# baek0203/multimodal_survival_prediction

Measured on AMD Instinct MI355X. Metric: patients/sec per epoch (training epoch of the K-fold job: fwd + Cox + gate entropy + bwd + clip + Adam; HBM-resident cohort, batches gathered on the device inside the timed region -- the same epoch fed from pinned host memory over PCIe: config.h2d), higher is better.
Workload: dtype f32

## Files before the change

include/mmsurv.h:

```cpp
#ifndef MMSURV_H
#define MMSURV_H
#include <stdint.h>
#include <stddef.h>

#ifndef HIP_INCLUDE_HIP_HIP_RUNTIME_API_H
typedef struct ihipStream_t* hipStream_t;
typedef struct ihipEvent_t* hipEvent_t;
#endif

#define MMS_OK 0
#define MMS_ERR_ARG (-1)
#define MMS_ERR_LAUNCH (-2)
#define MMS_MAX_GROUP 10

#ifdef __cplusplus
extern "C" {
#endif

typedef struct Dims3 { int D; int H; int W; } Dims3;

typedef struct MmsDnOpts {
    int out_features;
    int persist_b4;
    int persist_b3;
// ... 152 lines not shown
typedef struct MmsWgradMember {
    float* dw2;
    float* dw1;
    float* dgamma2; float* dbeta2;
    int model; int layer;
} MmsWgradMember;
typedef struct MmsWgradShape {
    int ld; int C0;
    int ms3; int ms1;
    int dw_layout;
    int count;
} MmsWgradShape;

typedef struct Conv1BwdP {
    const float* dyraw; int lddy;
    const float* y; int ldy;
    BnSrc bn_out; BnBwd bb_out; int has_bn_out;
    int M; int N;
    const float* x; int ldx; int K; BnSrc bn_in;
    const float* w;
    int pool; Dims3 in;
    float* dw;
    float* dbn; int lddbn;
    double* s1; double* s2;
    int msplit;
    float* dgamma_out; float* dbeta_out;
    int srep; int sstride;
    float* fuse_dx; int fuse_lddx; int fuse_accumulate;
    float* fuse_dgamma; float* fuse_dbeta;
    const unsigned* live;
} Conv1BwdP;

typedef struct BnBwdApplyP {
    const float* dbn; int lddbn;
    const float* x; int ldx;
    float* dx; int lddx;
    int M; int C; BnSrc bn; BnBwd bb; int accumulate;
    float* dgamma; float* dbeta;
    const unsigned* live;
} BnBwdApplyP;

typedef struct HeadBwdP {
    const float* dout; int lddout;
    const float* pooled;
    const float* slab; int ld; int C; int B; int V; BnSrc bn;
    const float* w; int N;
    float* dw; float* dbias;
    float* dgamma; float* dbeta;
    float* dslab; int ldd;
    double* ext_sums;
} HeadBwdP;

typedef struct PoolBwdP {
    const float* dslab; int ld;
    const uint8_t* argmax; Dims3 out; Dims3 in; int B;
    const float* y0; BnSrc bn;
    float* dbn;
    double* s1; double* s2;
    const int* coords;
    int srep; int sstride;
} PoolBwdP;

typedef struct Conv0BwdWP {
    const float* dbn; const float* y0; BnSrc bn; BnBwd bb;
    const float* x; Dims3 in; Dims3 out; const int* coords; int M;
    float* dw; int msplit;
    float* dgamma; float* dbeta;
    float* dw_rep; int nrep;
    const unsigned* live;
} Conv0BwdWP;

typedef struct Conv0BwdDataP {
    const float* dbn;
    BnSrc bn;
    const float* w;
    Dims3 in; Dims3 out;
    int M;
    float* dx;
} Conv0BwdDataP;

typedef struct FbConvP {
    const float* x; int Cin; Dims3 in; Dims3 out; int B;
    int has_bn; BnSrc bn;
    const float* w; const float* bias; int Cout;
    float* y;
    double* osum; double* osumsq;
    const float* dy;
    float* dw; float* dbias;
    float* dbn_in; double* s1; double* s2;
    int msplit;
} FbConvP;

typedef struct FbPoolP {
    const float* y; int C; int V; int B; BnSrc bn;
    float* out; int ldo;
    const float* dout; int lddout;
    float* dbn; double* s1; double* s2;
} FbPoolP;

typedef struct InProlog {
    int bn;
    const float* gamma; const float* beta;
    float* rmean; float* rvar; long long* nbt;
    float eps; float momentum;
    int train;
    float drop_p;
    const float* drop_mask;
    const uint32_t* rng;
    uint32_t stream_id;
} InProlog;

typedef struct LinearFwdP {
    const float* x; int ldx; int M; int K;
    InProlog pro;
    const float* w; const float* bias; int N;
    float* y; int ldy; int out_relu;
} LinearFwdP;

typedef struct LinearBwdP {
    const float* dy; int lddy;
    const float* y; int ldy;
    int out_relu;
    const float* x; int ldx; int M; int K; InProlog pro;
    const float* w; int N;
    float* dw; float* dbias;
    float* dx; int lddx;
    float* dgamma; float* dbeta;
} LinearBwdP;

typedef struct GateP {
    const float* feats; const float* mask; int M;
    const float* w1; const float* b1; const float* w2; const float* b2;
    float* hidden;
    float* gate;
    float* fused;
    const float* dfused;
    float ent_weight;
    const float* dgate_ext;
    float* dfeats;
    float* dw1; float* db1; float* dw2; float* db2;
    float* entropy;
} GateP;

typedef struct CoxP {
    const float* h; int ldh;
    const float* time; const float* event; const float* valid; int n;
    float scale;
    float* lse;
    float* dh; int lddh;
    float* out;
    int tie_mode;
    float* tie_frac;
} CoxP;

typedef struct CindexP {
    const float* h; const float* time; const float* event; int n;
    unsigned long long* counts;
} CindexP;

#define MMS_CBOOT_MAX_N 1048576
#define MMS_CBOOT_MAX_R 1048576
#define MMS_CBOOT_MAX_M 8
typedef struct CbootP {
    const int* hrank; int ldh; int M;
    const int* trank;
    const int* event;
    const int* stratum;
    int n;
    const signed char* w; int ldw; int R;
    long long* out;
    int pair_rule;
} CbootP;

#define MMS_GENE_SCREEN_MAX_G 4194240
typedef struct GeneScreenP {
    const float* x; int N; int ld;
    int G; int P;
    const int* off;
    const int* row;
    const double* coef;
    double* U; double* V;
} GeneScreenP;

#define MMS_COXNET_MAX_TOL 1.0
#define MMS_COXNET_MAX_ITER 100000000
typedef struct CoxnetP {
    const float* x; int N; int ld; int G;
    int nrow;
    const int* row; const int* event; const int* glast;
    int P;
    const int* mult;
    const double* lam; const double* alpha;
    const double* inv_scale;
    double* beta; double* trial; double* grad;
    double* f; double* step;
    int* iters; int* status;
    double* loss; double* nsum; double* kkt; double* obj;
    double* E; double* R;
    double* Gr;
    int* counter;
    double tol; int max_iter;
} CoxnetP;

#define MMS_LRSCAN_MAX_N 65535
#define MMS_LRSCAN_MAX_C 65535
#define MMS_LRSCAN_MAX_Q 16777215
typedef struct LogrankScanP {
    int n; int ldr; int Q;
    int maxc;
    const int* rank;
    const int* pflag;
    const double* coef;
    const int* coff;
    const int* cut;
    const int* cset;
    const int* at;
    double* chi2_max; int* arg_max; double* chi2_at;
    double* U; double* V;
    int* n_high; int* d_high;
    int ldo;
} LogrankScanP;

#define MMS_TD_MAX_H 64
#define MMS_TD_MAX_M 64
#define MMS_TD_MAX_N 4096
#define MMS_TD_MAX_R 16777215
typedef struct TdMetricsP {
    int n; int H; int M; int R;
    const int* trank; const int* event;
    const int* hcut;
    const int* rord; int ldr;
    const double* surv; int ldh;
    const signed char* w; int ldw;
    double* G; double* km;
    double* wcase; double* wctrl;
    double* brier; double* auc_num;
} TdMetricsP;

#define MMS_COXNEWTON_MAX_P 16
#define MMS_COXNEWTON_MAX_N 4096
#define MMS_COXNEWTON_MAX_S 64
#define MMS_COXNEWTON_MAX_Q 16777215
#define MMS_COXNEWTON_MAX_TOL 1e-3
#define MMS_COXNEWTON_MAX_ITER 1000
typedef struct CoxNewtonP {
    int n; int p; int R; int S;
    const double* x; int ldx;
    const int* event; const int* glast;
    const signed char* w; int ldw;
    const int* cmask;
    double tol; int max_iter; double beta_max;
    double* beta; double* se;
    double* loglik; double* loglik0;
    int* iters; int* status;
    double* info;
} CoxNewtonP;

typedef struct AdamP {
    float* p; float* g; float* m; float* v; long long n;
    const float* hyper;
    double* sumsq;
    float* step;
    const float* skip_flag;
    int adamw;
    float* acc; const float* cox_out; const float* entropy;
    int* rng;
    const long long* w2_off; float* const* w2_pack_b; float* const* w2_pack_f; int n_w2; uint64_t w2_fragmask;
} AdamP;

typedef struct LinBigP {
    const float* x; int ldx; int M; int K;
    const float* w; const float* bias; int N;
    float* y; int ldy; int out_relu;
    int has_bn; BnSrc bn;
    float* rmean; float* rvar; long long* nbt; float momentum;
    float drop_p; const float* drop_mask; const uint32_t* rng; uint32_t stream_id; int train;
    double* osum; double* osumsq;
    const float* dy; int lddy;
    float* dw; float* dbias; int msplit;
    int core_only;
    float* dbn; int lddbn;
    double* s1; double* s2;
    float* dx; int lddx;
    float* dgamma; float* dbeta;
} LinBigP;

typedef struct MixP {
    float* feats; int ld; int M;
    const float* mask; int ldm;
    int nseg;
    int seg_begin[4]; int seg_width[4];
    const float* bias[4];
    float* dfeats; int ldd;
    float* dbias[4];
} MixP;

typedef struct MoeP {
    int M; int F;
    int stage;
    const float* feats; int ldf;
    const float* mask; int ldm;
    const float* valid;
    float* valid_x;
    float* gin; int ldg;
    const float* h2; int ldh2;
    const float* w3; const float* b3;
// ... 46 lines not shown
} AffRec;
typedef struct AffP {
    const AffRec* rec;
    int stage_floats;
} AffP;

int mms_abi_sizeof(const char* name);
int mms_abi_version(void);

int mms_init_coords(int* coords, int B, int D, int H, int W, hipStream_t s);
int mms_conv0_fwd(const Conv0FwdP* p, hipStream_t s);
int mms_pool_fwd(const PoolFwdP* p, hipStream_t s);
int mms_conv1_fwd(const Conv1FwdP* p, hipStream_t s);
int mms_conv3_fwd(const Conv3FwdP* p, hipStream_t s);
int mms_head_fwd(const HeadFwdP* p, hipStream_t s);
int mms_conv3_bwd_data(const Conv3BwdDataP* p, hipStream_t s);
int mms_conv3_bwd_weight(const Conv3BwdWP* p, hipStream_t s);
int mms_conv1_bwd_data(const Conv1BwdP* p, hipStream_t s);
int mms_conv1_bwd_weight(const Conv1BwdP* p, hipStream_t s);
int mms_bn_bwd_apply(const BnBwdApplyP* p, hipStream_t s);
int mms_head_bwd(const HeadBwdP* p, hipStream_t s);
int mms_pool_bwd(const PoolBwdP* p, hipStream_t s);
int mms_conv0_bwd_weight(const Conv0BwdWP* p, hipStream_t s);
int mms_unpack_conv3_grads(const void* table_host, int nlayers, hipStream_t s);
int mms_pack_conv3(const float* w, float* wpf, float* wpb, hipStream_t s);
int mms_pack_conv3_frag(const float* w, float* wff, float* wfb, hipStream_t s);
int mms_pack_conv3_table(const void* table_dev, int nlayers, hipStream_t s);
int mms_bn_running_update(const void* table_dev, int n, float momentum, hipStream_t s);


int mms_fb_conv_fwd(const FbConvP* p, hipStream_t s);
int mms_fb_conv_bwd_w(const FbConvP* p, hipStream_t s);
int mms_fb_conv_bwd_x(const FbConvP* p, hipStream_t s);
int mms_fb_pool_fwd(const FbPoolP* p, hipStream_t s);
int mms_fb_pool_bwd(const FbPoolP* p, hipStream_t s);
int mms_fb_workspace_bytes(int B, int D, int H, int W, size_t* bytes);
int mms_fb_init(void* ws, int B, int D, int H, int W, const void* const* buffers, hipStream_t s);
int mms_fb_forward(void* ws, int B, int D, int H, int W, const float* x, const void* const* params,
                   const void* const* buffers, float* out, int ldo, int train, hipStream_t s);
int mms_fb_backward(void* ws, int B, int D, int H, int W, const float* x, const void* const* params,
                    const float* dout, int lddout, void* const* grads, hipStream_t s);
int mms_fb3_workspace_bytes(const int* widths, int B, int D, int H, int W, size_t* bytes);
int mms_fb3_init(void* ws, size_t ws_bytes, const int* widths, int B, int D, int H, int W, const void* const* buffers, hipStream_t s);
int mms_fb3_forward(void* ws, size_t ws_bytes, const int* widths, int B, int D, int H, int W, const float* x, const void* const* params,
                    const void* const* buffers, float* out, int ldo, int train, hipStream_t s);
int mms_fb3_backward(void* ws, size_t ws_bytes, const int* widths, int B, int D, int H, int W, const float* x, const void* const* params,
                     const float* dout, int lddout, void* const* grads, hipStream_t s);

int mms_conv0_bwd_data(const Conv0BwdDataP* p, hipStream_t s);
int mms_conv0_bwd_data_group(const Conv0BwdDataP* p, int ng, hipStream_t s);
int mms_dn121_input_grad(void* ws, int B, int D, int H, int W, const float* x, const void* const* params, const void* const* buffers,
                         const float* dout, int lddout, float* dx, const MmsDnOpts* opts, hipStream_t s);
int mms_fb3_input_grad(void* ws, size_t ws_bytes, const int* widths, int B, int D, int H, int W, const float* x, const void* const* params,
                       const void* const* buffers, const float* dout, int lddout, float* dx, hipStream_t s);
int mms_dn121_input_grad_group(int ng, void* const* ws, int B, int D, int H, int W, const float* const* x, const void* const* const* params,
                               const void* const* const* buffers, const float* const* dout, int lddout, float* const* dx,
                               const MmsDnOpts* opts, hipStream_t s);
int mms_fb3_input_grad_group(int ng, void* const* ws, size_t ws_bytes, const int* widths, int B, int D, int H, int W, const float* const* x,
                             const void* const* const* params, const void* const* const* buffers, const float* const* dout, int lddout,
                             float* const* dx, hipStream_t s);

typedef struct EnsP {
    const float* x[10];
    int K; size_t n;
    float* mean; float* spread;
} EnsP;
int mms_ensemble_reduce(const EnsP* p, hipStream_t s);

int mms_linear_fwd(const LinearFwdP* p, hipStream_t s);
int mms_linear_bwd(const LinearBwdP* p, hipStream_t s);
int mms_gate_fwd(const GateP* p, hipStream_t s);
int mms_gate_bwd(const GateP* p, hipStream_t s);
int mms_gate_entropy(const float* gate, int M, float scale, float* loss, float* dgate, hipStream_t s);
int mms_linear_big_fwd(const LinBigP* p, hipStream_t s);
int mms_linear_big_bwd_w(const LinBigP* p, hipStream_t s);
int mms_linear_big_bwd_x(const LinBigP* p, hipStream_t s);
int mms_bn1d_bwd_apply(const LinBigP* p, hipStream_t s);
int mms_missing_mix_fwd(const MixP* p, hipStream_t s);
int mms_missing_mix_bwd(const MixP* p, hipStream_t s);
int mms_cox_fwd_bwd(const CoxP* p, hipStream_t s);
int mms_moe_fwd(const MoeP* p, hipStream_t s);
int mms_moe_bwd(const MoeP* p, hipStream_t s);
int mms_cindex_counts(const CindexP* p, hipStream_t s);
int mms_cindex_boot(const CbootP* p, hipStream_t s);
int mms_gene_screen(const GeneScreenP* p, hipStream_t s);
int mms_logrank_scan(const LogrankScanP* p, hipStream_t s);
int mms_td_metrics(const TdMetricsP* p, hipStream_t s);
int mms_cox_newton(const CoxNewtonP* p, hipStream_t s);
int mms_coxnet_eval(const CoxnetP* p, hipStream_t s);
int mms_coxnet_iterate(const CoxnetP* p, int iters, hipStream_t s);
int mms_grad_sumsq(const AdamP* p, hipStream_t s);
int mms_clip_adam(const AdamP* p, hipStream_t s);
int mms_w2_pack(const AdamP* p, hipStream_t s);

int mms_ablation_build(void);
int mms_dn121_workspace_bytes(int B, int D, int H, int W, size_t* bytes);
int mms_dn121_region(int B, int D, int H, int W, const char* name, int index, size_t* off, size_t* bytes);
int mms_dn121_init(void* ws, int B, int D, int H, int W, const void* const* params, const void* const* buffers, const MmsDnOpts* opts, hipStream_t s);
int mms_dn121_w2_fragmask(int B, int D, int H, int W, const MmsDnOpts* opts, uint64_t* mask);
int mms_dn121_forward(void* ws, int B, int D, int H, int W, const float* x, const void* const* params,
                      const void* const* buffers, float* out, int ldo, int train, const MmsDnOpts* opts, hipStream_t s);
int mms_dn121_backward(void* ws, int B, int D, int H, int W, const float* x, const void* const* params,
                       const float* dout, int lddout, void* const* grads, const MmsDnOpts* opts, hipStream_t s);
typedef int (*mms_sync_fn)(void* user, double* base, int nrep, long rep_stride, int ncols, long pair_stride, hipStream_t s);
int mms_dn121_init_sync(void* ws, int B, int D, int H, int W, const void* const* params, const void* const* buffers, int bn_world,
                        const MmsDnOpts* opts, hipStream_t s);
int mms_dn121_forward_sync(void* ws, int B, int D, int H, int W, const float* x, const void* const* params,
                           const void* const* buffers, float* out, int ldo, int bn_world, mms_sync_fn hook, void* user,
                           const MmsDnOpts* opts, hipStream_t s);
int mms_dn121_backward_stage(void* ws, int B, int D, int H, int W, const float* x, const void* const* params,
                             const float* dout, int lddout, void* const* grads, int block_hi, int block_lo,
                             int bn_world, mms_sync_fn hook, void* user, const MmsDnOpts* opts, hipStream_t s);
int mms_head_bwd_sums(const HeadBwdP* p, hipStream_t s);
int mms_head_bwd_apply(const HeadBwdP* p, hipStream_t s);
int mms_dn121_backward_mt(void* ws, int B, int D, int H, int W, const float* x, const void* const* params,
                          const float* dout, int lddout, void* const* grads, const MmsDnOpts* opts, hipStream_t s, hipStream_t side,
                          hipEvent_t ev_fork, hipEvent_t ev_join);

int mms_ct_preprocess(const float* x, int inD, int inH, int inW, float* out, int oD, int oH, int oW, float* scratch, hipStream_t s);
int mms_rna_log_zscore(const float* counts, float* out, int n, int g, hipStream_t s);

int mms_conv0_fwd_group(const Conv0FwdP* p, int ng, const MmsDnOpts* opts, hipStream_t s);
int mms_conv0_fwd_group_zw(const Conv0FwdP* p, unsigned* const* zwords, int ng, const MmsDnOpts* opts, hipStream_t s);
int mms_pool_fwd_group(const PoolFwdP* p, int ng, hipStream_t s);
int mms_pool_act_group(const PoolActP* p, int ng, hipStream_t s);
int mms_conv1_fwd_group(const Conv1FwdP* p, int ng, const MmsDnOpts* opts, hipStream_t s);
int mms_conv3_fwd_group(const Conv3FwdP* p, int ng, const MmsDnOpts* opts, hipStream_t s);
int mms_head_fwd_group(const HeadFwdP* p, int ng, hipStream_t s);
int mms_conv3_bwd_data_group(const Conv3BwdDataP* p, int ng, const MmsDnOpts* opts, hipStream_t s);
int mms_conv3_bwd_weight_group(const Conv3BwdWP* p, int ng, const MmsDnOpts* opts, hipStream_t s);
int mms_conv3_bwd_weight_msplit(int M, int members, const MmsDnOpts* opts);
int mms_conv1_bwd_data_group(const Conv1BwdP* p, int ng, const MmsDnOpts* opts, hipStream_t s);
int mms_conv1_bwd_weight_group(const Conv1BwdP* p, int ng, hipStream_t s);
int mms_wgrad_tab_group(const MmsWgradModel* models, int nmodels, const MmsWgradMember* members, int nmembers,
                        const MmsWgradShape* shape, int which, hipStream_t s);
int mms_bn_bwd_apply_group(const BnBwdApplyP* p, int ng, hipStream_t s);
int mms_head_bwd_group(const HeadBwdP* p, int ng, hipStream_t s);
int mms_head_bwd_group_dup(const HeadBwdP* p, unsigned* const* live_out, const unsigned* const* zwords, int zbps, unsigned* const* dup_out,
                           int ng, hipStream_t s);
int mms_pool_bwd_group(const PoolBwdP* p, int ng, hipStream_t s);
int mms_conv0_bwd_weight_group(const Conv0BwdWP* p, int ng, const MmsDnOpts* opts, hipStream_t s);
int mms_pack_conv3_table_group(const void* const* tables_dev, int ng, int nlayers, hipStream_t s);
int mms_pack_conv3_table_group_ex(const void* const* tables_dev, int ng, int nlayers, uint64_t fragmask, hipStream_t s);
int mms_bn_running_update_group(const void* const* tables_dev, int ng, int n, float momentum, hipStream_t s);
int mms_missing_mix_fwd_group(const MixP* p, int ng, hipStream_t s);
int mms_missing_mix_bwd_group(const MixP* p, int ng, hipStream_t s);
int mms_gather_rows_group(const GatherP* p, int ng, hipStream_t s);
int mms_gather_aug_group(const GatherP* p, const AugP* a, int ng, hipStream_t s);
int mms_gather_affine_group(const GatherP* p, const AugP* a, const AffP* f, int ng, hipStream_t s);
int mms_unpack_conv3_grads_group(const float* const* scratch, float* const* const* dw, int ng, int nlayers, hipStream_t s);
int mms_zero_regions_group(void* const* regions_dev, int ng, size_t bytes, hipStream_t s);
int mms_linear_fwd_group(const LinearFwdP* p, int ng, hipStream_t s);
int mms_linear_bwd_group(const LinearBwdP* p, int ng, hipStream_t s);
int mms_gate_fwd_group(const GateP* p, int ng, hipStream_t s);
int mms_gate_bwd_group(const GateP* p, int ng, hipStream_t s);
int mms_cox_fwd_bwd_group(const CoxP* p, int ng, hipStream_t s);
int mms_moe_fwd_group(const MoeP* p, int ng, hipStream_t s);
int mms_moe_bwd_group(const MoeP* p, int ng, hipStream_t s);
int mms_grad_sumsq_group(const AdamP* p, int ng, hipStream_t s);
int mms_clip_adam_group(const AdamP* p, int ng, hipStream_t s);
int mms_w2_pack_group(const AdamP* p, int ng, hipStream_t s);
int mms_dn121_forward_group(int ng, void* const* ws, int B, int D, int H, int W, const float* const* x,
                            const void* const* const* params, const void* const* const* buffers, float* const* out,
                            int ldo, int train, const MmsDnOpts* opts, hipStream_t s);
int mms_dn121_backward_group(int ng, void* const* ws, int B, int D, int H, int W, const float* const* x,
                             const void* const* const* params, const float* const* dout, int lddout,
                             void* const* const* grads, const MmsDnOpts* opts, hipStream_t s);

int mms_fb_conv_fwd_group(const FbConvP* p, int ng, hipStream_t s);
int mms_fb_conv_bwd_w_group(const FbConvP* p, int ng, hipStream_t s);
int mms_fb_conv_bwd_x_group(const FbConvP* p, int ng, hipStream_t s);
int mms_fb_pool_fwd_group(const FbPoolP* p, int ng, hipStream_t s);
int mms_fb_pool_bwd_group(const FbPoolP* p, int ng, hipStream_t s);
int mms_fb_forward_group(int ng, void* const* ws, int B, int D, int H, int W, const float* const* x,
                         const void* const* const* params, const void* const* const* buffers, float* const* out,
                         int ldo, int train, hipStream_t s);
int mms_fb_backward_group(int ng, void* const* ws, int B, int D, int H, int W, const float* const* x,
                          const void* const* const* params, const float* const* dout, int lddout,
                          void* const* const* grads, hipStream_t s);
int mms_fb3_forward_group(int ng, void* const* ws, size_t ws_bytes, const int* widths, int B, int D, int H, int W, const float* const* x,
                          const void* const* const* params, const void* const* const* buffers, float* const* out,
                          int ldo, int train, hipStream_t s);
int mms_fb3_backward_group(int ng, void* const* ws, size_t ws_bytes, const int* widths, int B, int D, int H, int W, const float* const* x,
                           const void* const* const* params, const float* const* dout, int lddout,
                           void* const* const* grads, hipStream_t s);
int mms_img_tail_fwd_group(const FbPoolP* pool, const LinearFwdP* l1, const LinearFwdP* l2, int ng, hipStream_t s);
int mms_img_tail_bwd_group(const FbPoolP* pool, const LinearBwdP* l1, const LinearBwdP* l2, int ng, hipStream_t s);
int mms_img_forward_group(int ng, void* const* ws, size_t ws_bytes, const int* widths, int B, int D, int H, int W, const float* const* x,
                          const void* const* const* params, const void* const* const* buffers, float* const* out,
                          int ldo, int train, const LinearFwdP* l1, const LinearFwdP* l2, hipStream_t s);
int mms_img_backward_group(int ng, void* const* ws, size_t ws_bytes, const int* widths, int B, int D, int H, int W, const float* const* x,
                           const void* const* const* params, void* const* const* grads, const LinearBwdP* l1, const LinearBwdP* l2,
                           hipStream_t s);

#ifdef __cplusplus
}
#endif
#endif
```

multimodal_survival_prediction_amd/csrc/abi.hip:

```cpp
#include "common.h"
#include <string.h>

#define SZ(T) if (strcmp(name, #T) == 0) return (int)sizeof(T);
extern "C" int mms_abi_sizeof(const char* name) {
    SZ(Dims3) SZ(MmsDnOpts) SZ(BnSrc) SZ(BnBwd) SZ(Conv1FwdP) SZ(Conv3FwdP) SZ(Conv0FwdP) SZ(PoolFwdP) SZ(PoolActP) SZ(HeadFwdP)
    SZ(Conv3BwdDataP) SZ(Conv3BwdWP) SZ(Conv1BwdP) SZ(BnBwdApplyP) SZ(HeadBwdP) SZ(PoolBwdP) SZ(Conv0BwdWP) SZ(Conv0BwdDataP) SZ(InProlog) SZ(LinearFwdP) SZ(LinearBwdP) SZ(GateP) SZ(CoxP) SZ(CindexP) SZ(AdamP) SZ(FbConvP) SZ(FbPoolP) SZ(GatherP) SZ(AugRec) SZ(AugP) SZ(AffRec) SZ(AffP) SZ(MixP) SZ(LinBigP) SZ(MoeP) SZ(MmsWgradModel) SZ(MmsWgradMember) SZ(MmsWgradShape) SZ(EnsP) SZ(CbootP) SZ(GeneScreenP) SZ(CoxnetP) SZ(LogrankScanP) SZ(TdMetricsP) SZ(CoxNewtonP)
    return -1;
}
extern "C" int mms_abi_version(void) { return 3; }
extern "C" int mms_ablation_build(void) {
#if defined(MMS_ABLATE_STEP) || defined(MMS_ABLATE_SETUP) || defined(MMS_ABLATE_FLUSH) || defined(MMS_ABLATE_STATS) || defined(B4_TIMING) || defined(C3S_TIMING) || defined(C3M_TIMING)
    return 1;
#else
    return 0;
#endif
}
```

multimodal_survival_prediction_amd/csrc/heads.hip:

```cpp
#include "common.h"
#include "gather_rows.h"

template <int MM>
struct ColProlog {
    float xhat[MM], pre[MM], scale[MM];
    float mean, rstd, gamma;
    template <bool UPDATE_RUNNING>
    __device__ __forceinline__ void apply(const InProlog& pr, float (&x)[MM], int M, int k, int K) {
        if (pr.bn) {
            float mu, var;
            if (pr.train) {
                mu = 0;
#pragma unroll
                for (int m = 0; m < MM; ++m) if (m < M) mu += x[m];
                mu /= (float)M;
                var = 0;
#pragma unroll
                for (int m = 0; m < MM; ++m) if (m < M) { float d = x[m] - mu; var = fmaf(d, d, var); }
                var /= (float)M;
                if (UPDATE_RUNNING) {
                    const float unb = M > 1 ? var * (float)M / (float)(M - 1) : var;
                    pr.rmean[k] = (1.f - pr.momentum) * pr.rmean[k] + pr.momentum * mu;
                    pr.rvar[k] = (1.f - pr.momentum) * pr.rvar[k] + pr.momentum * unb;
                }
            } else {
                mu = pr.rmean[k]; var = pr.rvar[k];
            }
            mean = mu; rstd = 1.0f / sqrtf(var + pr.eps); gamma = pr.gamma[k];
            const float be = pr.beta[k];
#pragma unroll
            for (int m = 0; m < MM; ++m) {
                xhat[m] = (x[m] - mu) * rstd;
                pre[m] = fmaf(gamma, xhat[m], be);
                x[m] = fmaxf(pre[m], 0.f);
            }
        }
#pragma unroll
        for (int m = 0; m < MM; ++m) scale[m] = 1.f;
        if (pr.train && (pr.drop_mask || pr.drop_p > 0.f)) {
#pragma unroll
            for (int m = 0; m < MM; ++m) {
                if (m < M) {
                    scale[m] = pr.drop_mask ? pr.drop_mask[(size_t)m * K + k]
                                            : dropout_scale(pr.rng[0] + 0x9E3779B9u * pr.rng[1], pr.stream_id, (uint32_t)(m * K + k), pr.drop_p);
                    x[m] *= scale[m];
                }
            }
        }
    }
};

template <int MM, bool KS4>
__global__ __launch_bounds__(256) void linear_fwd_kernel(const Grp<LinearFwdP> grp) {
    const LinearFwdP& p = grp.p[blockIdx.z];
    __shared__ float red[4][MM];
    const int lane = threadIdx.x & 63, wave = threadIdx.x >> 6, n = KS4 ? (int)blockIdx.x : (int)blockIdx.x * 4 + wave;
    if (n >= p.N) return;
    constexpr int KSTEP = KS4 ? 256 : 64;
    const bool upd = (n == 0) && p.pro.bn && p.pro.train;
    float acc[MM];
#pragma unroll
    for (int m = 0; m < MM; ++m) acc[m] = 0.f;
    int kstart = lane + (KS4 ? 64 * wave : 0);
    const float* __restrict__ wr = p.w + (size_t)n * p.K;
    const float* __restrict__ xr = p.x;
    const bool plain = !p.pro.bn && !(p.pro.train && (p.pro.drop_mask || p.pro.drop_p > 0.f));
    constexpr int NU = MM <= 4 ? 8 : (MM <= 8 ? 4 : 2);
    for (; kstart + KSTEP * (NU - 1) < p.K; kstart += KSTEP * NU) {
        float w4[NU], x4[NU][MM];
#pragma unroll
        for (int u = 0; u < NU; ++u) {
            w4[u] = wr[kstart + KSTEP * u];
#pragma unroll
            for (int m = 0; m < MM; ++m) x4[u][m] = m < p.M ? xr[(size_t)m * p.ldx + kstart + KSTEP * u] : 0.f;
        }
#pragma unroll
        for (int u = 0; u < NU; ++u) {
            if (!plain) {
                ColProlog<MM> cp;
                if (upd) cp.template apply<true>(p.pro, x4[u], p.M, kstart + KSTEP * u, p.K); else cp.template apply<false>(p.pro, x4[u], p.M, kstart + KSTEP * u, p.K);
            }
#pragma unroll
            for (int m = 0; m < MM; ++m) acc[m] = fmaf(w4[u], x4[u][m], acc[m]);
        }
    }
    for (int k = kstart; k < p.K; k += KSTEP) {
        float x[MM];
#pragma unroll
        for (int m = 0; m < MM; ++m) x[m] = m < p.M ? xr[(size_t)m * p.ldx + k] : 0.f;
        ColProlog<MM> cp;
        if (upd) cp.template apply<true>(p.pro, x, p.M, k, p.K); else cp.template apply<false>(p.pro, x, p.M, k, p.K);
        const float w = wr[k];
#pragma unroll
        for (int m = 0; m < MM; ++m) acc[m] = fmaf(w, x[m], acc[m]);
    }
    if (upd && lane == 0 && (!KS4 || wave == 0) && p.pro.nbt) *p.pro.nbt += 1;
    const float b = p.bias ? p.bias[n] : 0.f;
#pragma unroll
    for (int m = 0; m < MM; ++m) acc[m] = wave_sum(acc[m]);
    if constexpr (KS4) {
        if (lane == 0) {
#pragma unroll
            for (int m = 0; m < MM; ++m) red[wave][m] = acc[m];
        }
        __syncthreads();
        if (wave != 0) return;
#pragma unroll
        for (int m = 0; m < MM; ++m) acc[m] = red[0][m] + red[1][m] + red[2][m] + red[3][m];
    }
    if (lane == 0) {
#pragma unroll
        for (int m = 0; m < MM; ++m)
            if (m < p.M) {
                const float v = acc[m] + b;
                p.y[(size_t)m * p.ldy + n] = p.out_relu ? fmaxf(v, 0.f) : v;
            }
    }
}

template <int MM>
static int launch_linear_fwd(const Grp<LinearFwdP>& a, int ng, hipStream_t s) {
    if (a.p[0].K >= 2048) MMS_LAUNCH((linear_fwd_kernel<MM, true>), dim3(a.p[0].N, 1, ng), dim3(256), 0, s, a);
    else MMS_LAUNCH((linear_fwd_kernel<MM, false>), dim3((a.p[0].N + 3) / 4, 1, ng), dim3(256), 0, s, a);
    return mms_check_launch();
}
extern "C" int mms_linear_fwd_group(const LinearFwdP* pp, int ng, hipStream_t s) {
    Grp<LinearFwdP> a;
    if (!grp_fill(a, pp, ng, 1)) return MMS_ERR_ARG;
    const LinearFwdP& p = *pp;
    if (p.M <= 0 || p.M > 32 || p.N <= 0 || p.K <= 0) return MMS_ERR_ARG;
    if (p.pro.bn && p.pro.train && p.M < 2) return MMS_ERR_ARG;
    for (int g = 1; g < ng; ++g) {
        const LinearFwdP& q = pp[g];
        if (q.M != p.M || q.N != p.N || q.K != p.K || q.pro.bn != p.pro.bn || q.pro.train != p.pro.train) return MMS_ERR_ARG;
    }
    if (p.M <= 4) return launch_linear_fwd<4>(a, ng, s);
    if (p.M <= 8) return launch_linear_fwd<8>(a, ng, s);
    if (p.M <= 16) return launch_linear_fwd<16>(a, ng, s);
    return launch_linear_fwd<32>(a, ng, s);
}
MMS_SINGLE(mms_linear_fwd, LinearFwdP)

template <int MM, bool KS4>
__global__ __launch_bounds__(256) void linear_bwd_w_kernel(const Grp<LinearBwdP> grp) {
    const LinearBwdP& p = grp.p[blockIdx.z];
    const int lane = threadIdx.x & 63, wave = threadIdx.x >> 6, n = KS4 ? (int)blockIdx.x : (int)blockIdx.x * 4 + wave;
    if (n >= p.N) return;
    constexpr int KSTEP = KS4 ? 256 : 64;
    float dz[MM], db = 0.f;
#pragma unroll
    for (int m = 0; m < MM; ++m) {
        float g = 0.f;
        if (m < p.M) {
            g = p.dy[(size_t)m * p.lddy + n];
            if (p.out_relu && !(p.y[(size_t)m * p.ldy + n] > 0.f)) g = 0.f;
        }
        dz[m] = g; db += g;
    }
    if (lane == 0 && (!KS4 || wave == 0) && p.dbias) p.dbias[n] += db;
    constexpr int NU = MM <= 4 ? 8 : 2;
    float* __restrict__ dwr = p.dw + (size_t)n * p.K;
    const float* __restrict__ xr = p.x;
    int k0 = lane + (KS4 ? 64 * wave : 0);
    for (; k0 + KSTEP * (NU - 1) < p.K; k0 += KSTEP * NU) {
        float d0[NU], xx[NU][MM];
#pragma unroll
        for (int u = 0; u < NU; ++u) {
            d0[u] = dwr[k0 + KSTEP * u];
#pragma unroll
            for (int m = 0; m < MM; ++m) xx[u][m] = m < p.M ? xr[(size_t)m * p.ldx + k0 + KSTEP * u] : 0.f;
        }
#pragma unroll
        for (int u = 0; u < NU; ++u) {
            ColProlog<MM> cp;
            cp.template apply<false>(p.pro, xx[u], p.M, k0 + KSTEP * u, p.K);
            float a = 0.f;
#pragma unroll
            for (int m = 0; m < MM; ++m) a = fmaf(dz[m], xx[u][m], a);
            dwr[k0 + KSTEP * u] = d0[u] + a;
        }
    }
    for (int k = k0; k < p.K; k += KSTEP) {
        float x[MM];
#pragma unroll
        for (int m = 0; m < MM; ++m) x[m] = m < p.M ? p.x[(size_t)m * p.ldx + k] : 0.f;
        ColProlog<MM> cp;
        cp.template apply<false>(p.pro, x, p.M, k, p.K);
        float a = 0.f;
#pragma unroll
        for (int m = 0; m < MM; ++m) a = fmaf(dz[m], x[m], a);
        p.dw[(size_t)n * p.K + k] += a;
    }
}

template <int MM>
__global__ __launch_bounds__(256) void linear_bwd_x_kernel(const Grp<LinearBwdP> grp) {
    const LinearBwdP& p = grp.p[blockIdx.z];
    __shared__ float dzs[MM][128];
    __shared__ float red[3][MM][64];
    const int lane = threadIdx.x & 63, wave = threadIdx.x >> 6;
    const int k = blockIdx.x * 64 + lane;
    const int N = p.N, K = p.K;
    const float* __restrict__ wk = p.w + (k < K ? k : K - 1);
    float acc[MM];
#pragma unroll
    for (int m = 0; m < MM; ++m) acc[m] = 0.f;
    for (int nb = 0; nb < N; nb += 128) {
        __syncthreads();
        for (int idx = threadIdx.x; idx < MM * 128; idx += 256) {
            const int m = idx >> 7, n = nb + (idx & 127);
            float g = 0.f;
            if (m < p.M && n < N) {
                g = p.dy[(size_t)m * p.lddy + n];
                if (p.out_relu && !(p.y[(size_t)m * p.ldy + n] > 0.f)) g = 0.f;
            }
            dzs[m][idx & 127] = g;
        }
        __syncthreads();
        if (nb + 32 * wave < N) {
#pragma unroll
            for (int h = 0; h < 2; ++h) {
                float wv[16];
#pragma unroll
                for (int j = 0; j < 16; ++j) {
                    const int n = nb + 32 * wave + 16 * h + j;
                    wv[j] = wk[(size_t)(n < N ? n : N - 1) * K];
                }
#pragma unroll
                for (int j = 0; j < 16; ++j)
#pragma unroll
                    for (int m = 0; m < MM; ++m) acc[m] = fmaf(dzs[m][32 * wave + 16 * h + j], wv[j], acc[m]);
            }
        }
    }
    if (wave > 0) {
#pragma unroll
        for (int m = 0; m < MM; ++m) red[wave - 1][m][lane] = acc[m];
    }
    __syncthreads();
    if (wave > 0 || k >= K) return;
#pragma unroll
    for (int m = 0; m < MM; ++m) acc[m] += red[0][m][lane] + red[1][m][lane] + red[2][m][lane];
    float x[MM];
#pragma unroll
    for (int m = 0; m < MM; ++m) x[m] = m < p.M ? p.x[(size_t)m * p.ldx + k] : 0.f;
    ColProlog<MM> cp;
    cp.template apply<false>(p.pro, x, p.M, k, p.K);
    float dxv[MM];
    if (p.pro.bn) {
        float s1 = 0.f, s2 = 0.f, dpre[MM];
#pragma unroll
        for (int m = 0; m < MM; ++m) {
            dpre[m] = (m < p.M && cp.pre[m] > 0.f) ? acc[m] * cp.scale[m] : 0.f;
            s1 += dpre[m]; s2 = fmaf(dpre[m], cp.xhat[m], s2);
        }
        if (p.dgamma) { p.dgamma[k] += s2; p.dbeta[k] += s1; }
        const float gr = cp.gamma * cp.rstd, m1 = s1 / (float)p.M, m2 = s2 / (float)p.M;
#pragma unroll
        for (int m = 0; m < MM; ++m)
            dxv[m] = p.pro.train ? gr * (dpre[m] - m1 - cp.xhat[m] * m2) : gr * dpre[m];
    } else {
#pragma unroll
        for (int m = 0; m < MM; ++m) dxv[m] = acc[m] * cp.scale[m];
    }
#pragma unroll
    for (int m = 0; m < MM; ++m) if (m < p.M) p.dx[(size_t)m * p.lddx + k] = dxv[m];
}

template <int MM>
static int launch_linear_bwd(const Grp<LinearBwdP>& a, int ng, hipStream_t s) {
    const LinearBwdP& p = a.p[0];
    if (p.dw) {
        if (p.K >= 2048) MMS_LAUNCH((linear_bwd_w_kernel<MM, true>), dim3(p.N, 1, ng), dim3(256), 0, s, a);
        else MMS_LAUNCH((linear_bwd_w_kernel<MM, false>), dim3((p.N + 3) / 4, 1, ng), dim3(256), 0, s, a);
    }
    if (p.dx) MMS_LAUNCH(linear_bwd_x_kernel<MM>, dim3((p.K + 63) / 64, 1, ng), dim3(256), 0, s, a);
    return mms_check_launch();
}
extern "C" int mms_linear_bwd_group(const LinearBwdP* pp, int ng, hipStream_t s) {
    Grp<LinearBwdP> a;
    if (!grp_fill(a, pp, ng, 1)) return MMS_ERR_ARG;
    const LinearBwdP& p = *pp;
    if (p.M <= 0 || p.M > 32 || p.N <= 0 || p.K <= 0) return MMS_ERR_ARG;
    for (int g = 1; g < ng; ++g) {
        const LinearBwdP& q = pp[g];
        if (q.M != p.M || q.N != p.N || q.K != p.K || (q.dw == nullptr) != (p.dw == nullptr) || (q.dx == nullptr) != (p.dx == nullptr)) return MMS_ERR_ARG;
    }
    if (p.M <= 4) return launch_linear_bwd<4>(a, ng, s);
    if (p.M <= 8) return launch_linear_bwd<8>(a, ng, s);
    if (p.M <= 16) return launch_linear_bwd<16>(a, ng, s);
    return launch_linear_bwd<32>(a, ng, s);
}
MMS_SINGLE(mms_linear_bwd, LinearBwdP)

#define GATE_F 288
#define GATE_IN 291
__device__ __forceinline__ int gate_seg(int t) { return t < 128 ? 0 : (t < 256 ? 1 : 2); }

__global__ __launch_bounds__(256) void gate_fwd_kernel(const Grp<GateP> grp) {
    const GateP& p = grp.p[blockIdx.z];
    __shared__ float G[GATE_IN + 1], h[64], g[3];
    const int m = blockIdx.x, t = threadIdx.x, lane = t & 63, wave = t >> 6;
    for (int i = t; i < GATE_IN; i += 256)
        G[i] = i < GATE_F ? p.feats[(size_t)m * GATE_F + i] * p.mask[m * 3 + gate_seg(i)] : p.mask[m * 3 + (i - GATE_F)];
    __syncthreads();
    for (int j = wave * 16; j < wave * 16 + 16; ++j) {
        float a = 0.f;
        for (int k = lane; k < GATE_IN; k += 64) a = fmaf(p.w1[j * GATE_IN + k], G[k], a);
        a = wave_sum(a);
        if (lane == 0) { h[j] = fmaxf(a + p.b1[j], 0.f); p.hidden[m * 64 + j] = h[j]; }
    }
    __syncthreads();
    if (wave == 0) {
        float l[3];
#pragma unroll
        for (int c = 0; c < 3; ++c) l[c] = wave_sum(p.w2[c * 64 + lane] * h[lane]) + p.b2[c];
        if (lane == 0) {
            const float mx = fmaxf(l[0], fmaxf(l[1], l[2]));
            const float e0 = expf(l[0] - mx), e1 = expf(l[1] - mx), e2 = expf(l[2] - mx), inv = 1.f / (e0 + e1 + e2);
            g[0] = e0 * inv; g[1] = e1 * inv; g[2] = e2 * inv;
            float ent = 0.f;
#pragma unroll
            for (int c = 0; c < 3; ++c) { p.gate[m * 3 + c] = g[c]; ent += g[c] * logf(g[c] + 1e-8f); }
            if (p.entropy) atomicAdd(p.entropy, ent / (float)p.M);
        }
    }
    __syncthreads();
    for (int i = t; i < GATE_F; i += 256) p.fused[(size_t)m * GATE_F + i] = G[i] * g[gate_seg(i)];
}

__global__ __launch_bounds__(256) void gate_bwd_kernel(const Grp<GateP> grp) {
    const GateP& p = grp.p[blockIdx.z];
    __shared__ float G[GATE_IN + 1], h[64], g[3], dgs[3], dl[3], dhp[64], red[4][3];
    const int m = blockIdx.x, t = threadIdx.x, lane = t & 63, wave = t >> 6;
    for (int i = t; i < GATE_IN; i += 256)
        G[i] = i < GATE_F ? p.feats[(size_t)m * GATE_F + i] * p.mask[m * 3 + gate_seg(i)] : p.mask[m * 3 + (i - GATE_F)];
    if (t < 64) h[t] = p.hidden[m * 64 + t];
    if (t < 3) g[t] = p.gate[m * 3 + t];
    __syncthreads();
    float part[3] = {0.f, 0.f, 0.f};
    for (int i = t; i < GATE_F; i += 256) part[gate_seg(i)] += p.dfused[(size_t)m * GATE_F + i] * G[i];
#pragma unroll
    for (int c = 0; c < 3; ++c) { float v = wave_sum(part[c]); if (lane == 0) red[wave][c] = v; }
    __syncthreads();
    if (t == 0) {
        float dg[3], dot = 0.f;
#pragma unroll
        for (int c = 0; c < 3; ++c) {
            dg[c] = red[0][c] + red[1][c] + red[2][c] + red[3][c];
            if (p.ent_weight != 0.f) dg[c] += p.ent_weight / (float)p.M * (logf(g[c] + 1e-8f) + g[c] / (g[c] + 1e-8f));
            if (p.dgate_ext) dg[c] += p.dgate_ext[m * 3 + c];
            dot += g[c] * dg[c];
        }
#pragma unroll
        for (int c = 0; c < 3; ++c) { dl[c] = g[c] * (dg[c] - dot); atomicAdd(&p.db2[c], dl[c]); }
    }
    __syncthreads();
    if (t < 64) {
        float dh = 0.f;
#pragma unroll
        for (int c = 0; c < 3; ++c) { dh = fmaf(dl[c], p.w2[c * 64 + t], dh); atomicAdd(&p.dw2[c * 64 + t], dl[c] * h[t]); }
        dhp[t] = h[t] > 0.f ? dh : 0.f;
        atomicAdd(&p.db1[t], dhp[t]);
    }
    __syncthreads();
    for (int idx = t; idx < 64 * GATE_IN; idx += 256) {
        const int j = idx / GATE_IN, k = idx % GATE_IN;
        atomicAdd(&p.dw1[idx], dhp[j] * G[k]);
    }
    for (int i = t; i < GATE_F; i += 256) {
        float dG = 0.f;
        for (int j = 0; j < 64; ++j) dG = fmaf(dhp[j], p.w1[j * GATE_IN + i], dG);
        const int sg = gate_seg(i);
        p.dfeats[(size_t)m * GATE_F + i] = (p.dfused[(size_t)m * GATE_F + i] * g[sg] + dG) * p.mask[m * 3 + sg];
    }
}
#define GATE_TR 8
template <bool SPLIT>
__global__ __launch_bounds__(256) void gate_bwd_tiled_kernel(const Grp<GateP> grp) {
    const GateP& p = grp.p[blockIdx.z];
    __shared__ float G[GATE_IN + 1], h[64], g[3], dl[3], dhp[64], red[4][3];
    const int t = threadIdx.x, lane = t & 63, wave = t >> 6;
    const int role = SPLIT ? (int)blockIdx.y : 0;
    const bool do_acc = !SPLIT || role == 0, do_feats = !SPLIT || role > 0;
    int m_lo = blockIdx.x * GATE_TR, m_hi = m_lo + GATE_TR < p.M ? m_lo + GATE_TR : p.M;
    if (SPLIT && role > 0) { m_lo += role - 1; if (m_lo >= m_hi) return; m_hi = m_lo + 1; }
    const bool two = t < GATE_IN - 256;
    float a0[64], a1[64];
#pragma unroll
    for (int j = 0; j < 64; ++j) { a0[j] = 0.f; a1[j] = 0.f; }
    float ab1 = 0.f, aw2[3] = {0.f, 0.f, 0.f}, ab2[3] = {0.f, 0.f, 0.f};
    for (int m = m_lo; m < m_hi; ++m) {
        __syncthreads();
        for (int i = t; i < GATE_IN; i += 256)
            G[i] = i < GATE_F ? p.feats[(size_t)m * GATE_F + i] * p.mask[m * 3 + gate_seg(i)] : p.mask[m * 3 + (i - GATE_F)];
        if (t < 64) h[t] = p.hidden[m * 64 + t];
        if (t < 3) g[t] = p.gate[m * 3 + t];
        __syncthreads();
        float part[3] = {0.f, 0.f, 0.f};
        for (int i = t; i < GATE_F; i += 256) part[gate_seg(i)] += p.dfused[(size_t)m * GATE_F + i] * G[i];
#pragma unroll
        for (int c = 0; c < 3; ++c) { float v = wave_sum(part[c]); if (lane == 0) red[wave][c] = v; }
        __syncthreads();
        if (t == 0) {
            float dg[3], dot = 0.f;
#pragma unroll
            for (int c = 0; c < 3; ++c) {
                dg[c] = red[0][c] + red[1][c] + red[2][c] + red[3][c];
                if (p.ent_weight != 0.f) dg[c] += p.ent_weight / (float)p.M * (logf(g[c] + 1e-8f) + g[c] / (g[c] + 1e-8f));
                if (p.dgate_ext) dg[c] += p.dgate_ext[m * 3 + c];
                dot += g[c] * dg[c];
            }
#pragma unroll
            for (int c = 0; c < 3; ++c) { dl[c] = g[c] * (dg[c] - dot); ab2[c] += dl[c]; }
        }
        __syncthreads();
        if (t < 64) {
            float dh = 0.f;
#pragma unroll
            for (int c = 0; c < 3; ++c) { dh = fmaf(dl[c], p.w2[c * 64 + t], dh); aw2[c] = fmaf(dl[c], h[t], aw2[c]); }
            dhp[t] = h[t] > 0.f ? dh : 0.f;
            ab1 += dhp[t];
        }
        __syncthreads();
        if (do_acc) {
            const float g0 = G[t], g1 = two ? G[256 + t] : 0.f;
#pragma unroll
            for (int j = 0; j < 64; ++j) { const float d = dhp[j]; a0[j] = fmaf(d, g0, a0[j]); a1[j] = fmaf(d, g1, a1[j]); }
        }
        if (do_feats)
            for (int i = t; i < GATE_F; i += 256) {
                float dG = 0.f;
                for (int j = 0; j < 64; ++j) dG = fmaf(dhp[j], p.w1[j * GATE_IN + i], dG);
                const int sg = gate_seg(i);
                p.dfeats[(size_t)m * GATE_F + i] = (p.dfused[(size_t)m * GATE_F + i] * g[sg] + dG) * p.mask[m * 3 + sg];
            }
    }
    if (!do_acc) return;
#pragma unroll
    for (int j = 0; j < 64; ++j) {
        atomicAdd(&p.dw1[j * GATE_IN + t], a0[j]);
        if (two) atomicAdd(&p.dw1[j * GATE_IN + 256 + t], a1[j]);
    }
    if (t < 64) {
        atomicAdd(&p.db1[t], ab1);
#pragma unroll
        for (int c = 0; c < 3; ++c) atomicAdd(&p.dw2[c * 64 + t], aw2[c]);
    }
    if (t == 0) {
#pragma unroll
        for (int c = 0; c < 3; ++c) atomicAdd(&p.db2[c], ab2[c]);
    }
}
__global__ void gate_entropy_kernel(const float* gate, int M, float scale, float* loss, float* dgate) {
    const int m = blockIdx.x * 64 + threadIdx.x;
    float e = 0.f;
    if (m < M) {
#pragma unroll
        for (int c = 0; c < 3; ++c) {
            const float g = gate[m * 3 + c];
            e += g * logf(g + 1e-8f);
            if (dgate) dgate[m * 3 + c] = scale / (float)M * (logf(g + 1e-8f) + g / (g + 1e-8f));
        }
    }
    e = wave_sum(e);
    if (threadIdx.x == 0 && loss) atomicAdd(loss, e / (float)M);
}
extern "C" int mms_gate_entropy(const float* gate, int M, float scale, float* loss, float* dgate, hipStream_t s) {
    if (M <= 0) return MMS_ERR_ARG;
    MMS_LAUNCH(gate_entropy_kernel, dim3((M + 63) / 64), dim3(64), 0, s, gate, M, scale, loss, dgate);
    return mms_check_launch();
}

static bool gate_group(Grp<GateP>& a, const GateP* pp, int ng) {
    if (!grp_fill(a, pp, ng, 1) || pp->M <= 0) return false;
    for (int g = 1; g < ng; ++g) if (pp[g].M != pp->M) return false;
    return true;
}
extern "C" int mms_gate_fwd_group(const GateP* pp, int ng, hipStream_t s) {
    Grp<GateP> a;
    if (!gate_group(a, pp, ng)) return MMS_ERR_ARG;
    MMS_LAUNCH(gate_fwd_kernel, dim3(pp->M, 1, ng), dim3(256), 0, s, a);
    return mms_check_launch();
}
extern "C" int mms_gate_bwd_group(const GateP* pp, int ng, hipStream_t s) {
    Grp<GateP> a;
    if (!gate_group(a, pp, ng)) return MMS_ERR_ARG;
    if (pp->M <= GATE_TR) MMS_LAUNCH(gate_bwd_tiled_kernel<true>, dim3(1, 1 + pp->M, ng), dim3(256), 0, s, a);
    else if (pp->M > 32) MMS_LAUNCH(gate_bwd_tiled_kernel<false>, dim3((pp->M + GATE_TR - 1) / GATE_TR, 1, ng), dim3(256), 0, s, a);
    else MMS_LAUNCH(gate_bwd_kernel, dim3(pp->M, 1, ng), dim3(256), 0, s, a);
    return mms_check_launch();
}
MMS_SINGLE(mms_gate_fwd, GateP)
MMS_SINGLE(mms_gate_bwd, GateP)

__device__ __forceinline__ bool cox_valid(const CoxP& p, int i) { return p.valid == nullptr || p.valid[i] != 0.f; }

__global__ __launch_bounds__(256) void cox_lse_kernel(const Grp<CoxP> grp) {
    const CoxP& p = grp.p[blockIdx.z];
    const int lane = threadIdx.x & 63, i = blockIdx.x * 4 + (threadIdx.x >> 6);
    if (i >= p.n) return;
    if (!cox_valid(p, i)) { if (lane == 0) { p.lse[i] = 0.f; if (p.tie_mode == 1) p.tie_frac[i] = -1.f; } return; }
    const float ti = p.time[i];
    float mx = -INFINITY;
    for (int j = lane; j < p.n; j += 64)
        if (cox_valid(p, j) && p.time[j] >= ti) mx = fmaxf(mx, p.h[(size_t)j * p.ldh]);
    mx = wave_max(mx);
    float s = 0.f;
    if (p.tie_mode != 1) {
        for (int j = lane; j < p.n; j += 64)
            if (cox_valid(p, j) && p.time[j] >= ti) s += expf(p.h[(size_t)j * p.ldh] - mx);
        s = wave_sum(s);
        if (lane == 0) p.lse[i] = mx + logf(s);
        return;
    }
    float st = 0.f, m = 0.f, l = 0.f;
    for (int j = lane; j < p.n; j += 64)
        if (cox_valid(p, j)) {
            const float tj = p.time[j];
            if (tj >= ti) {
                const float e = expf(p.h[(size_t)j * p.ldh] - mx);
                s += e;
                if (tj == ti && p.event[j] != 0.f) { st += e; m += 1.f; l += j < i ? 1.f : 0.f; }
            }
        }
    s = wave_sum(s); st = wave_sum(st); m = wave_sum(m); l = wave_sum(l);
    if (lane == 0) {
        const bool ev = p.event[i] != 0.f;
        const float f = ev ? l / m : 0.f;
        p.lse[i] = mx + logf(s - f * st);
        p.tie_frac[i] = ev ? f : -1.f;
    }
}

__global__ __launch_bounds__(256) void cox_grad_kernel(const Grp<CoxP> grp) {
    const CoxP& p = grp.p[blockIdx.z];
    __shared__ float red[8];
    const int lane = threadIdx.x & 63, wave = threadIdx.x >> 6, k = blockIdx.x * 4 + wave;
    const bool efron = p.tie_mode == 1;
    float nv = 0.f, ne = 0.f, ls = 0.f, nd = 0.f;
    for (int j = threadIdx.x; j < p.n; j += 256)
        if (cox_valid(p, j)) {
            nv += 1.f;
            if (p.event[j] != 0.f) {
                ne += 1.f; ls += p.h[(size_t)j * p.ldh] - p.lse[j];
                if (efron && p.tie_frac[j] == 0.f) nd += 1.f;
            }
        }
    nv = wave_sum(nv); ne = wave_sum(ne); ls = wave_sum(ls); nd = wave_sum(nd);
    if (lane == 0) { red[wave] = nv; red[4 + wave] = ne; }
    __syncthreads();
    nv = red[0] + red[1] + red[2] + red[3]; ne = red[4] + red[5] + red[6] + red[7];
    __syncthreads();
    if (lane == 0) { red[wave] = ls; red[4 + wave] = nd; }
    __syncthreads();
    ls = red[0] + red[1] + red[2] + red[3]; nd = red[4] + red[5] + red[6] + red[7];
    const bool usable = nv >= 2.f && ne > 0.f;
    const float denom = efron ? nd : ne + 1e-8f;
    if (blockIdx.x == 0 && threadIdx.x == 0) {
        p.out[0] = usable ? -ls / denom : 0.f;
        p.out[1] = usable ? 1.f : 0.f;
    }
    if (k >= p.n || p.dh == nullptr) return;
    float gsum = 0.f;
    if (usable && cox_valid(p, k)) {
        const float tk = p.time[k], hk = p.h[(size_t)k * p.ldh];
        const bool ek = p.event[k] != 0.f;
        for (int i = lane; i < p.n; i += 64)
            if (cox_valid(p, i) && p.event[i] != 0.f && p.time[i] <= tk) {
                float w = 1.f;
                if (efron && ek && p.time[i] == tk) w -= p.tie_frac[i];
                gsum += w * expf(hk - p.lse[i]);
            }
        gsum = wave_sum(gsum);
        if (lane == 0) p.dh[(size_t)k * p.lddh] = -p.scale * ((ek ? 1.f : 0.f) - gsum) / denom;
    } else if (lane == 0) {
        p.dh[(size_t)k * p.lddh] = 0.f;
    }
}
extern "C" int mms_cox_fwd_bwd_group(const CoxP* pp, int ng, hipStream_t s) {
    Grp<CoxP> a;
    if (!grp_fill(a, pp, ng, 1)) return MMS_ERR_ARG;
    const CoxP& p = *pp;
    for (int g = 0; g < ng; ++g)
        if (pp[g].n != p.n || pp[g].n <= 0 || !pp[g].lse || !pp[g].out || pp[g].tie_mode < 0 || pp[g].tie_mode > 1 || (pp[g].tie_mode == 1 && !pp[g].tie_frac)) return MMS_ERR_ARG;
    MMS_LAUNCH(cox_lse_kernel, dim3((p.n + 3) / 4, 1, ng), dim3(256), 0, s, a);
    MMS_LAUNCH(cox_grad_kernel, dim3((p.n + 3) / 4, 1, ng), dim3(256), 0, s, a);
    return mms_check_launch();
}
MMS_SINGLE(mms_cox_fwd_bwd, CoxP)

__global__ __launch_bounds__(256) void cindex_kernel(const CindexP p) {
    const int lane = threadIdx.x & 63, i = blockIdx.x * 4 + (threadIdx.x >> 6);
    if (i >= p.n || p.event[i] != 1.f) return;
    const float ti = p.time[i], hi = p.h[i];
    unsigned conc = 0, tied = 0, perm = 0;
    for (int j = lane; j < p.n; j += 64)
        if (p.time[j] > ti) {
            ++perm;
            const float hj = p.h[j];
            conc += hi > hj; tied += hi == hj;
        }
#pragma unroll
    for (int o = 32; o > 0; o >>= 1) { conc += __shfl_xor(conc, o, 64); tied += __shfl_xor(tied, o, 64); perm += __shfl_xor(perm, o, 64); }
    if (lane == 0) {
        atomicAdd(&p.counts[0], (unsigned long long)conc);
        atomicAdd(&p.counts[1], (unsigned long long)tied);
        atomicAdd(&p.counts[2], (unsigned long long)perm);
    }
}
extern "C" int mms_cindex_counts(const CindexP* pp, hipStream_t s) {
    if (pp->n <= 0) return MMS_ERR_ARG;
    MMS_LAUNCH(cindex_kernel, dim3((pp->n + 3) / 4), dim3(256), 0, s, *pp);
    return mms_check_launch();
}

__global__ __launch_bounds__(256) void grad_sumsq_kernel(const Grp<AdamP> grp) {
    const AdamP& p = grp.p[blockIdx.z];
    __shared__ double red[4];
    const long long n4 = p.n >> 2, stride = (long long)gridDim.x * 256;
    float a = 0.f, a1 = 0.f, a2 = 0.f, a3 = 0.f;
    long long i = (long long)blockIdx.x * 256 + threadIdx.x;
    for (; i + 3 * stride < n4; i += 4 * stride) {
        const float4 g0 = ((const float4*)p.g)[i], g1 = ((const float4*)p.g)[i + stride], g2 = ((const float4*)p.g)[i + 2 * stride],
                     g3 = ((const float4*)p.g)[i + 3 * stride];
        a = fmaf(g0.x, g0.x, a); a = fmaf(g0.y, g0.y, a); a = fmaf(g0.z, g0.z, a); a = fmaf(g0.w, g0.w, a);
        a1 = fmaf(g1.x, g1.x, a1); a1 = fmaf(g1.y, g1.y, a1); a1 = fmaf(g1.z, g1.z, a1); a1 = fmaf(g1.w, g1.w, a1);
        a2 = fmaf(g2.x, g2.x, a2); a2 = fmaf(g2.y, g2.y, a2); a2 = fmaf(g2.z, g2.z, a2); a2 = fmaf(g2.w, g2.w, a2);
        a3 = fmaf(g3.x, g3.x, a3); a3 = fmaf(g3.y, g3.y, a3); a3 = fmaf(g3.z, g3.z, a3); a3 = fmaf(g3.w, g3.w, a3);
    }
    for (; i < n4; i += stride) {
        const float4 g = ((const float4*)p.g)[i];
        a = fmaf(g.x, g.x, a); a = fmaf(g.y, g.y, a); a = fmaf(g.z, g.z, a); a = fmaf(g.w, g.w, a);
    }
    a += a1 + a2 + a3;
    if (blockIdx.x == 0 && threadIdx.x < (p.n & 3)) { const float g = p.g[(n4 << 2) + threadIdx.x]; a = fmaf(g, g, a); }
    const double t = block_sum_d((double)a, red);
    if (threadIdx.x == 0) {
        atomicAdd(p.sumsq, t);
        if (blockIdx.x == 0) {
            if (p.skip_flag == nullptr || *p.skip_flag != 0.f) p.step[0] += 1.f;
            if (p.acc) {
                if (p.cox_out) { p.acc[0] += p.cox_out[0] * p.cox_out[1]; p.acc[1] += p.cox_out[1]; }
                if (p.entropy) p.acc[2] += p.entropy[0];
                p.acc[3] += 1.f;
            }
            if (p.rng) p.rng[1] += 1;
        }
    }
}
constexpr int W2N = 32 * 27 * 128;
__global__ __launch_bounds__(256) void clip_adam_kernel(const Grp<AdamP> grp) {
    const AdamP& p = grp.p[blockIdx.z];
    __shared__ float c[6];
    if (p.skip_flag != nullptr && *p.skip_flag == 0.f) return;
    if (threadIdx.x == 0) {
        const double lr = p.hyper[0], b1 = p.hyper[1], b2 = p.hyper[2], wd = p.hyper[4], maxn = p.hyper[5];
        const double t = p.step[0];
        const double norm = sqrt(*p.sumsq);
        double coef = maxn / (norm + 1e-6);
        if (coef > 1.0) coef = 1.0;
        if (maxn <= 0.0) coef = 1.0;
        const double bc1 = 1.0 - pow(b1, t), bc2 = 1.0 - pow(b2, t);
        c[0] = (float)coef; c[1] = (float)(lr / bc1); c[2] = (float)(1.0 / sqrt(bc2));
        c[3] = (float)(1.0 - lr * wd); c[4] = (float)wd;
    }
    __syncthreads();
    const float coef = c[0], step_size = c[1], inv_sqrt_bc2 = c[2], decay = c[3], wd = c[4];
    const float b1 = p.hyper[1], b2 = p.hyper[2], eps = p.hyper[3];
    const long long stride = (long long)gridDim.x * 256;
    __shared__ long long vp[64];
    const int nw = p.n_w2;
    if ((int)threadIdx.x < nw) vp[threadIdx.x] = p.w2_off[threadIdx.x] - (long long)threadIdx.x * W2N;
    if (nw) __syncthreads();
    const long long nv = p.n - (long long)nw * W2N;
    for (long long j = (long long)blockIdx.x * 256 + threadIdx.x; j < nv; j += stride) {
        int lo = 0, hi = nw;
        while (lo < hi) { const int mid = (lo + hi) >> 1; if (vp[mid] <= j) lo = mid + 1; else hi = mid; }
        const long long i = j + (long long)lo * W2N;
        float w = p.p[i], g = p.g[i] * coef;
        if (p.adamw) w *= decay; else g = fmaf(wd, w, g);
        const float m = fmaf(b1, p.m[i], (1.f - b1) * g);
        const float v = fmaf(b2, p.v[i], (1.f - b2) * g * g);
        p.m[i] = m; p.v[i] = v;
        p.p[i] = w - step_size * m / (sqrtf(v) * inv_sqrt_bc2 + eps);
    }
}

constexpr int W2P = 132;

template <bool UPDATE>
__global__ __launch_bounds__(256) void w2_adam_pack_kernel(const Grp<AdamP> grp) {
    const AdamP& p = grp.p[blockIdx.z];
    const int tap = blockIdx.x, layer = blockIdx.y, tid = threadIdx.x;
    __shared__ __attribute__((aligned(16))) float t[32 * W2P];
    __shared__ float c[6];
    if (UPDATE) {
        if (p.skip_flag != nullptr && *p.skip_flag == 0.f) return;
        if (tid == 0) {
            const double lr = p.hyper[0], b1 = p.hyper[1], b2 = p.hyper[2], wd = p.hyper[4], maxn = p.hyper[5];
            const double st = p.step[0];
            const double norm = sqrt(*p.sumsq);
            double coef = maxn / (norm + 1e-6);
            if (coef > 1.0) coef = 1.0;
            if (maxn <= 0.0) coef = 1.0;
            const double bc1 = 1.0 - pow(b1, st), bc2 = 1.0 - pow(b2, st);
            c[0] = (float)coef; c[1] = (float)(lr / bc1); c[2] = (float)(1.0 / sqrt(bc2));
            c[3] = (float)(1.0 - lr * wd); c[4] = (float)wd;
        }
        __syncthreads();
    }
    const size_t base = (size_t)p.w2_off[layer];
    float4 w4[4];
    size_t off[4];
#pragma unroll
    for (int j = 0; j < 4; ++j) {
        const int idx4 = tid + 256 * j, co = idx4 >> 5, c4 = idx4 & 31;
        off[j] = base + ((size_t)co * 27 + tap) * 128 + 4 * c4;
        w4[j] = *(const float4*)(p.p + off[j]);
    }
    if (UPDATE) {
        float4 g4[4], m4[4], v4[4];
#pragma unroll
        for (int j = 0; j < 4; ++j) { g4[j] = *(const float4*)(p.g + off[j]); m4[j] = *(const float4*)(p.m + off[j]); v4[j] = *(const float4*)(p.v + off[j]); }
        const float coef = c[0], step_size = c[1], inv_sqrt_bc2 = c[2], decay = c[3], wd = c[4];
        const float b1 = p.hyper[1], b2 = p.hyper[2], eps = p.hyper[3];
        auto upd = [&](float& w, float g, float& m, float& v) {
            g *= coef;
            if (p.adamw) w *= decay; else g = fmaf(wd, w, g);
            m = fmaf(b1, m, (1.f - b1) * g);
            v = fmaf(b2, v, (1.f - b2) * g * g);
            w = w - step_size * m / (sqrtf(v) * inv_sqrt_bc2 + eps);
        };
#pragma unroll
        for (int j = 0; j < 4; ++j) {
            upd(w4[j].x, g4[j].x, m4[j].x, v4[j].x); upd(w4[j].y, g4[j].y, m4[j].y, v4[j].y);
            upd(w4[j].z, g4[j].z, m4[j].z, v4[j].z); upd(w4[j].w, g4[j].w, m4[j].w, v4[j].w);
            *(float4*)(p.p + off[j]) = w4[j]; *(float4*)(p.m + off[j]) = m4[j]; *(float4*)(p.v + off[j]) = v4[j];
        }
    }
#pragma unroll
    for (int j = 0; j < 4; ++j) {
        const int idx4 = tid + 256 * j, co = idx4 >> 5, c4 = idx4 & 31;
        *(float4*)(t + co * W2P + 4 * c4) = w4[j];
    }
    __syncthreads();
    const bool frag = (p.w2_fragmask >> layer) & 1ull;
    float4* pb = (float4*)p.w2_pack_b[layer];
    if (frag) {
        float4* dst = pb + (size_t)tap * 1024;
#pragma unroll
        for (int j = 0; j < 4; ++j) {
            const int idx4 = tid + 256 * j, q = idx4 >> 6, lane = idx4 & 63;
            const int cin = ((q >> 1) << 4) | (lane & 15), co0 = ((q & 1) << 4) | ((lane >> 4) << 2);
            dst[idx4] = make_float4(t[co0 * W2P + cin], t[(co0 + 1) * W2P + cin], t[(co0 + 2) * W2P + cin], t[(co0 + 3) * W2P + cin]);
        }
        float4* df = (float4*)p.w2_pack_f[layer] + (size_t)tap * 1024;
#pragma unroll
        for (int j = 0; j < 4; ++j) {
            const int idx4 = tid + 256 * j, q = idx4 >> 6, lane = idx4 & 63;
            const int c4 = ((q >> 1) << 2) | (lane >> 4), co = ((q & 1) << 4) | (lane & 15);
            df[idx4] = *(const float4*)(t + co * W2P + 4 * c4);
        }
    } else {
#pragma unroll
        for (int j = 0; j < 4; ++j) {
            const int idx4 = tid + 256 * j, cin = idx4 >> 3, co0 = (idx4 & 7) << 2;
            pb[((size_t)cin * 27 + tap) * 8 + (idx4 & 7)] =
                make_float4(t[co0 * W2P + cin], t[(co0 + 1) * W2P + cin], t[(co0 + 2) * W2P + cin], t[(co0 + 3) * W2P + cin]);
        }
    }
}



static bool adam_group(Grp<AdamP>& a, const AdamP* pp, int ng) {
    if (!grp_fill(a, pp, ng, 1) || pp->n <= 0) return false;
    for (int g = 0; g < ng; ++g) {
        const AdamP& p = pp[g];
        if (p.n != pp->n || p.n_w2 != pp->n_w2 || p.w2_fragmask != pp->w2_fragmask || p.n_w2 < 0 || p.n_w2 > 64) return false;
        if (p.n_w2 && (!p.w2_off || !p.w2_pack_b || (p.w2_fragmask && !p.w2_pack_f) || (((uintptr_t)p.p | (uintptr_t)p.g | (uintptr_t)p.m | (uintptr_t)p.v) & 15))) return false;
    }
    return true;
}
extern "C" int mms_grad_sumsq_group(const AdamP* pp, int ng, hipStream_t s) {
    Grp<AdamP> a;
    if (!adam_group(a, pp, ng)) return MMS_ERR_ARG;
    long long blocks = (pp->n / 16 + 255) / 256;
    if (blocks > 1024) blocks = 1024;
    if (blocks < 1) blocks = 1;
    MMS_LAUNCH(grad_sumsq_kernel, dim3((unsigned)blocks, 1, ng), dim3(256), 0, s, a);
    return mms_check_launch();
}
extern "C" int mms_clip_adam_group(const AdamP* pp, int ng, hipStream_t s) {
    Grp<AdamP> a;
    if (!adam_group(a, pp, ng)) return MMS_ERR_ARG;
    long long blocks = (pp->n + 255) / 256;
    if (blocks > 4096) blocks = 4096;
    MMS_LAUNCH(clip_adam_kernel, dim3((unsigned)blocks, 1, ng), dim3(256), 0, s, a);
    if (pp->n_w2 > 0) MMS_LAUNCH(w2_adam_pack_kernel<true>, dim3(27, pp->n_w2, ng), dim3(256), 0, s, a);
    return mms_check_launch();
}
extern "C" int mms_w2_pack_group(const AdamP* pp, int ng, hipStream_t s) {
    Grp<AdamP> a;
    if (!adam_group(a, pp, ng)) return MMS_ERR_ARG;
    if (pp->n_w2 > 0) MMS_LAUNCH(w2_adam_pack_kernel<false>, dim3(27, pp->n_w2, ng), dim3(256), 0, s, a);
    return mms_check_launch();
}
MMS_SINGLE(mms_grad_sumsq, AdamP)
MMS_SINGLE(mms_clip_adam, AdamP)
MMS_SINGLE(mms_w2_pack, AdamP)

__global__ __launch_bounds__(256) void gather_rows_kernel(const Grp<GatherP> grp) {
    const GatherP& p = grp.p[blockIdx.z];
    const int b = blockIdx.y;
    if (b >= p.B) return;
    const long long row = p.idx[b];
    const int t0 = blockIdx.x * 256 + threadIdx.x, stride = gridDim.x * 256;
    for (int s = 0; s < p.nsrc; ++s) {
        const float* src = p.src[s] + (size_t)row * p.src_ld[s];
        float* dst = p.dst[s] + (size_t)b * p.dst_ld[s];
        const int w = p.width[s];
        const bool absent = p.present[s] && p.present[s][(size_t)row * p.present_ld[s]] == 0.f;
        if ((w & 3) == 0 && (((uintptr_t)src | (uintptr_t)dst) & 15) == 0) {
            if (absent) { for (int i = t0; i < (w >> 2); i += stride) ((float4*)dst)[i] = make_float4(0.f, 0.f, 0.f, 0.f); }
            else {
                int i = t0;
                for (; i + 3 * stride < (w >> 2); i += 4 * stride) {
                    const float4 a = ((const float4*)src)[i], b = ((const float4*)src)[i + stride], c = ((const float4*)src)[i + 2 * stride],
                                 d = ((const float4*)src)[i + 3 * stride];
                    ((float4*)dst)[i] = a; ((float4*)dst)[i + stride] = b; ((float4*)dst)[i + 2 * stride] = c; ((float4*)dst)[i + 3 * stride] = d;
                }
                for (; i < (w >> 2); i += stride) ((float4*)dst)[i] = ((const float4*)src)[i];
            }
        } else {
            for (int i = t0; i < w; i += stride) dst[i] = absent ? 0.f : src[i];
        }
    }
}
extern "C" int mms_gather_rows_group(const GatherP* pp, int ng, hipStream_t s) {
    Grp<GatherP> a;
    if (!grp_fill(a, pp, ng, 1)) return MMS_ERR_ARG;
    int wmax = 0;
    for (int g = 0; g < ng; ++g) {
        const GatherP& q = pp[g];
        if (q.B != pp->B || q.B <= 0 || !q.idx || q.nsrc < 1 || q.nsrc > 8) return MMS_ERR_ARG;
        for (int i = 0; i < q.nsrc; ++i) {
            if (!q.src[i] || !q.dst[i] || q.width[i] <= 0) return MMS_ERR_ARG;
            if (q.width[i] > wmax) wmax = q.width[i];
        }
    }
    int blocks = (wmax / 4 + 1023) / 1024;
    if (blocks < 1) blocks = 1;
    if (blocks > 64) blocks = 64;
    MMS_LAUNCH(gather_rows_kernel, dim3(blocks, pp->B, ng), dim3(256), 0, s, a);
    return mms_check_launch();
}

#define AUG_TILE4 1024

__global__ __launch_bounds__(256) void gather_aug_kernel(const Grp<GatherP> grp, const AugGrp ag) {
    __shared__ float4 tile[AUG_TILE4];
    const GatherP& p = grp.p[blockIdx.z];
    const AugK& k = ag.k[blockIdx.z];
    const int b = blockIdx.y;
    if (b >= p.B) return;
    const long long row = p.idx[b];
    const AugRec r = k.rec[b];
    const int t0 = blockIdx.x * 256 + threadIdx.x, stride = gridDim.x * 256;
    const bool ident_i = r.scale == 1.f && r.offset == 0.f;
    const bool ident = ident_i && (r.flip & 7) == 0 && r.dz == 0 && r.dy == 0 && r.dx == 0;
    for (int s = 0; s < p.nsrc; ++s) {
        const float* src;
        float* dst;
        if (gather_plain_source(p, k.meta, r.drop, s, row, b, ident, t0, stride, src, dst)) continue;
        const int w = p.width[s];
        const int D = ag.D, H = ag.H, W = ag.W;
        const int dz = max(-D, min(D, r.dz)), dy = max(-H, min(H, r.dy)), dx = max(-W, min(W, r.dx));
        const bool fD = r.flip & 1, fH = r.flip & 2, fW = r.flip & 4;
        if ((W & 3) == 0 && W <= 4 * AUG_TILE4 && (((uintptr_t)src | (uintptr_t)dst) & 15) == 0) {
            const int W4 = W >> 2, LT = AUG_TILE4 / W4, nlines = D * H, ntiles = (nlines + LT - 1) / LT;
            for (int t = blockIdx.x; t < ntiles; t += gridDim.x) {
                const int l0 = t * LT, n4 = min(LT, nlines - l0) * W4;
                float4 v[4];
#pragma unroll
                for (int u = 0; u < 4; ++u) {
                    const int j = threadIdx.x + u * 256;
                    v[u] = make_float4(0.f, 0.f, 0.f, 0.f);
                    if (j < n4) {
                        const int l = l0 + j / W4, xq = j - (j / W4) * W4;
                        const int z = l / H, y = l - z * H;
                        const int sz = (fD ? D - 1 - z : z) - dz, sy = (fH ? H - 1 - y : y) - dy;
                        if (sz >= 0 && sz < D && sy >= 0 && sy < H)
                            v[u] = ((const float4*)src)[(size_t)(sz * H + sy) * W4 + xq];
                    }
                }
#pragma unroll
                for (int u = 0; u < 4; ++u) { const int j = threadIdx.x + u * 256; if (j < n4) tile[j] = v[u]; }
                __syncthreads();
                const float* tf = (const float*)tile;
#pragma unroll
                for (int u = 0; u < 4; ++u) {
                    const int j = threadIdx.x + u * 256;
                    if (j < n4) {
                        const int ll = j / W4, x0 = (j - ll * W4) * 4;
                        float o[4];
#pragma unroll
                        for (int e = 0; e < 4; ++e) {
                            const int x = x0 + e, sx = (fW ? W - 1 - x : x) - dx;
                            const float q = (sx >= 0 && sx < W) ? tf[ll * W + sx] : 0.f;
                            o[e] = ident_i ? q : fmaf(r.scale, q, r.offset);
                        }
                        ((float4*)dst)[(size_t)l0 * W4 + j] = make_float4(o[0], o[1], o[2], o[3]);
                    }
                }
                __syncthreads();
            }
        } else {
            for (int i = t0; i < w; i += stride) {
                const int x = i % W, l = i / W, y = l % H, z = l / H;
                const int sz = (fD ? D - 1 - z : z) - dz, sy = (fH ? H - 1 - y : y) - dy, sx = (fW ? W - 1 - x : x) - dx;
                const float q = (sz >= 0 && sz < D && sy >= 0 && sy < H && sx >= 0 && sx < W) ? src[((size_t)sz * H + sy) * W + sx] : 0.f;
                dst[i] = ident_i ? q : fmaf(r.scale, q, r.offset);
            }
        }
    }
}
extern "C" int mms_gather_aug_group(const GatherP* pp, const AugP* aa, int ng, hipStream_t s) {
    Grp<GatherP> a;
    if (!grp_fill(a, pp, ng, 1) || !aa) return MMS_ERR_ARG;
    AugGrp ag = {};
    int blocks = 0;
    if (!gather_aug_args(pp, aa, ng, ag, blocks)) return MMS_ERR_ARG;
    MMS_LAUNCH(gather_aug_kernel, dim3(blocks, pp->B, ng), dim3(256), 0, s, a, ag);
    return mms_check_launch();
}

__global__ __launch_bounds__(256) void missing_mix_kernel(const Grp<MixP> grp, int bwd) {
    const MixP& p = grp.p[blockIdx.z];
    const int j = blockIdx.x * 256 + threadIdx.x;
    int s = -1;
    for (int t = 0; t < p.nseg; ++t) if (j >= p.seg_begin[t] && j < p.seg_begin[t] + p.seg_width[t]) s = t;
    if (s < 0) return;
    const int jl = j - p.seg_begin[s];
    if (!bwd) {
        const float b = p.bias[s][jl];
// ... 37 lines not shown
```

multimodal_survival_prediction_amd/engine.py:

```python
import ctypes
import os

import torch
import torch.nn as nn

from . import _lib, ops

_S = _lib.structs



def check_train_batch(B, bn_world=1):
    if B * max(int(bn_world), 1) <= 1:
        raise ValueError("Expected more than 1 value per channel when training: a batch of 1 patient cannot be normalised by the "
                         "heads' BatchNorm1d layers (torch raises the same in the reference's train_epoch; choose a batch size / "
                         "fold split without a tail of 1)")

class _Lin:

    def __init__(self, lin, src, dst, out_relu, pro_bn=None, pro_drop=None, need_dx=True):
        self.lin, self.src, self.dst, self.out_relu = lin, src, dst, out_relu
        self.pro_bn, self.pro_drop, self.need_dx = pro_bn, pro_drop, need_dx


# ... 387 lines not shown
            P.gate = ops.gate_params(P.buf["feats"], P.mask, g1.weight, g1.bias, g2.weight, g2.bias, P.hidden, P.gatew,
                                     P.buf["fused"], P.dbuf["fused"], self.ent_weight, P.dbuf["feats"],
                                     gmap[id(g1.weight)], gmap[id(g1.bias)], gmap[id(g2.weight)], gmap[id(g2.bias)],
                                     self.entropy)
        P.mix = None
        if prog.get("mix") is not None:
            mx = prog["mix"]
            P.mask2 = torch.ones(B, len(mx["segs"]), device=dev)
            M = _S()["MixP"]()
            fe, dfe = P.buf["feats"], P.dbuf["feats"]
            M.feats, M.ld, M.M = fe.data_ptr(), fe.stride(0), B
            M.mask, M.ldm, M.nseg = P.mask2.data_ptr(), P.mask2.stride(0), len(mx["segs"])
            M.dfeats, M.ldd = dfe.data_ptr(), dfe.stride(0)
            for i, ((b0, w), bias) in enumerate(zip(mx["segs"], mx["biases"])):
                M.seg_begin[i], M.seg_width[i] = b0, w
                M.bias[i], M.dbias[i] = bias.data_ptr(), gmap[id(bias)].data_ptr()
            P.mix = M
        P.moe = None
        if prog.get("moe") is not None:
            self._plan_moe(P, gmap)
        hz = P.buf["hz"]
        ens_valid = P.valid_x[0] if P.moe is not None else P.valid
        P.cox = _S()["CoxP"](hz.data_ptr(), hz.stride(0), P.time.data_ptr(), P.event.data_ptr(), ens_valid.data_ptr(), B, 1.0,
                             P.lse.data_ptr(), P.dbuf["hz"].data_ptr(), P.dbuf["hz"].stride(0), P.cox_out.data_ptr(), self.tie_mode,
                             P.tie_frac.data_ptr())
        P.cox_eval_out = torch.zeros(2, device=self.device)
        P.cox_eval = _S()["CoxP"](hz.data_ptr(), hz.stride(0), P.time.data_ptr(), P.event.data_ptr(), ens_valid.data_ptr(), B, 1.0,
                                  P.lse.data_ptr(), None, 1, P.cox_eval_out.data_ptr(), self.tie_mode, P.tie_frac.data_ptr())
        book = dict(acc=self.acc, cox_out=P.cox_out, entropy=self.entropy, rng=self.rng)
        w2 = self.w2 if (self.w2 is not None and self.w2["fragmask"] is not None) else None
        if self.w2 is not None and w2 is None:
            raise RuntimeError("create the engine's first plan with the encoder (packed conv2 storage needs the volume size)")
        P.adam = ops.adam_params(self.flat, self.gflat, self.m, self.v, self.hyper, self.sumsq, self.step_count,
                                 None, self.adamw, w2=w2, **book)
        P.adam_skip = ops.adam_params(self.flat, self.gflat, self.m, self.v, self.hyper, self.sumsq, self.step_count,
                                      P.cox_out[1:], self.adamw, w2=w2, **book)
        P.graphs = {}
        self.plans[key] = P
        return P

    def _plan_moe(self, P, gmap):
        mo, B, dev, S = self.prog["moe"], P.B, self.device, _S()
        F = mo["F"]
        P.gatew = torch.zeros(B, 3, device=dev)
        P.fused = torch.zeros(B, F, device=dev)
        P.valid_x = torch.ones(4, B, device=dev)
        P.cox_outs = torch.zeros(4, 2, device=dev)
        P.lse4, P.frac4 = torch.zeros(4, B, device=dev), torch.zeros(4, B, device=dev)
        fe, dfe, hz, dhz = P.buf["feats"], P.dbuf["feats"], P.buf["hz"], P.dbuf["hz"]
        gin, dgin, h2, dh2 = P.buf["gin"], P.dbuf["gin"], P.buf["g2"], P.dbuf["g2"]
        out, ens = mo["out"], mo["ensemble"]

        def block(stage):
            q = S["MoeP"]()
            q.M, q.F, q.stage = B, F, stage
            q.feats, q.ldf, q.mask, q.ldm = fe.data_ptr(), fe.stride(0), P.mask.data_ptr(), P.mask.stride(0)
            q.valid, q.valid_x = P.valid.data_ptr(), P.valid_x.data_ptr()
            q.gin, q.ldg, q.h2, q.ldh2 = gin.data_ptr(), gin.stride(0), h2.data_ptr(), h2.stride(0)
            q.w3, q.b3 = out.weight.data_ptr(), out.bias.data_ptr()
            for e, L in enumerate(mo["experts"]):
                q.wx[e], q.bx[e] = L.weight.data_ptr(), L.bias.data_ptr()
                q.dwx[e], q.dbx[e] = gmap[id(L.weight)].data_ptr(), gmap[id(L.bias)].data_ptr()
            q.we, q.be = ens.weight.data_ptr(), ens.bias.data_ptr()
            q.hz, q.ldhz, q.gate, q.fused = hz.data_ptr(), hz.stride(0), P.gatew.data_ptr(), P.fused.data_ptr()
            q.dhz, q.lddhz, q.dh2, q.lddh2 = dhz.data_ptr(), dhz.stride(0), dh2.data_ptr(), dh2.stride(0)
            q.dgin, q.lddg, q.dfeats, q.lddf = dgin.data_ptr(), dgin.stride(0), dfe.data_ptr(), dfe.stride(0)
            q.dw3, q.db3 = gmap[id(out.weight)].data_ptr(), gmap[id(out.bias)].data_ptr()
            q.dwe, q.dbe = gmap[id(ens.weight)].data_ptr(), gmap[id(ens.bias)].data_ptr()
            q.cox_outs, q.expert_weight, q.loss_out = P.cox_outs.data_ptr(), self.expert_weight, P.cox_out.data_ptr()
            return q
        P.moe = [block(0), block(1)]
        P.moe_bwd = [block(0), block(1)]
        lam = self.expert_weight
        cox = (S["CoxP"] * 4)()
        for c in range(4):
            valid = P.valid_x[c]
            cox[c] = S["CoxP"](hz[:, c].data_ptr(), hz.stride(0), P.time.data_ptr(), P.event.data_ptr(), valid.data_ptr(), B,
                               1.0 if c == 0 else lam, P.lse4[c].data_ptr(), dhz[:, c].data_ptr(), dhz.stride(0), P.cox_outs[c].data_ptr(),
                               self.tie_mode, P.frac4[c].data_ptr())
        P.cox4 = cox

    def _cox_step(self, P):
        if P.moe is not None:
            _lib.check(self.lib.mms_cox_fwd_bwd_group(P.cox4, 4, ops.stream()), "mms_cox_fwd_bwd_group")
        else:
            _lib.check(self.lib.mms_cox_fwd_bwd(ctypes.byref(P.cox), ops.stream()), "mms_cox_fwd_bwd")

    def _plan_big(self, P, gmap):
        prog, B, dev = self.prog, P.B, self.device
        S, ptr = _S()["LinBigP"], ops.ptr
        widths = {L.src: L.lin.in_features for L in prog["lins"] if L.pro_bn is not None}
        off, o = {}, 0
        for name, k in widths.items():
            off[name] = o
            o += 4 * k
        P.big_stats = torch.zeros(max(o, 1), dtype=torch.float64, device=dev)
        P.big_dbn = torch.zeros(B, max(list(widths.values()) + [4]), device=dev)
        st = lambda name, j: P.big_stats[off[name] + j * widths[name]:]
        P.big_lin = {True: [], False: []}
        for i, L in enumerate(prog["lins"]):
            (xs, xo), (ys, yo) = L.src, L.dst
            for what, name, co in (("source", xs, xo), ("destination", ys, yo)):
                if co % 4 != 0 or (co and P.buf[name].stride(0) % 4 != 0):
                    raise RuntimeError("large-batch path: %s column offset %d of buffer '%s' (pitch %d floats) of layer %d is not 16-byte "
                                       "aligned; feature widths must be multiples of 4" % (what, co, name, P.buf[name].stride(0), i))
            x, y = P.buf[xs][:, xo:], P.buf[ys][:, yo:]
            K, N = L.lin.in_features, L.lin.out_features
            for train in (True, False):
                q = S()
                q.x, q.ldx, q.M, q.K = x.data_ptr(), x.stride(0), B, K
                q.w, q.bias, q.N = L.lin.weight.data_ptr(), L.lin.bias.data_ptr(), N
                q.y, q.ldy, q.out_relu = y.data_ptr(), y.stride(0), 1 if L.out_relu else 0
                q.train = 1 if train else 0
                q.drop_p = float(L.pro_drop.p) if L.pro_drop is not None else 0.0
                q.drop_mask, q.rng, q.stream_id = ptr(self.dropout_masks.get(i)), self.rng.data_ptr(), i + 1
                bn = L.pro_bn
                if bn is not None:
                    q.has_bn = 1
                    q.bn.sum, q.bn.sumsq = st(L.src, 0).data_ptr(), st(L.src, 1).data_ptr()
                    q.bn.rmean, q.bn.rvar = bn.running_mean.data_ptr(), bn.running_var.data_ptr()
                    q.bn.gamma, q.bn.beta = bn.weight.data_ptr(), bn.bias.data_ptr()
                    q.bn.inv_count, q.bn.eps, q.bn.train, q.bn.nrep, q.bn.rep_stride = 1.0 / B, float(bn.eps), q.train, 1, 0
                    q.rmean, q.rvar, q.nbt = bn.running_mean.data_ptr(), bn.running_var.data_ptr(), bn.num_batches_tracked.data_ptr()
                    q.momentum = float(bn.momentum)
                if train and L.dst in widths:
                    q.osum, q.osumsq = st(L.dst, 0).data_ptr(), st(L.dst, 1).data_ptr()
                if train:
                    dy = P.dbuf[ys][:, yo:]
                    q.dy, q.lddy = dy.data_ptr(), dy.stride(0)
                    q.dw, q.dbias = gmap[id(L.lin.weight)].data_ptr(), gmap[id(L.lin.bias)].data_ptr()
                    tiles = ((N + 63) // 64) * ((K + 63) // 64)
                    q.msplit = max(1, min((512 + tiles - 1) // tiles, (B + 63) // 64))
                    if L.need_dx:
                        dx = P.dbuf[xs][:, xo:]
                        if bn is not None:
                            q.dbn, q.lddbn = P.big_dbn.data_ptr(), P.big_dbn.stride(0)
                            q.s1, q.s2 = st(L.src, 2).data_ptr(), st(L.src, 3).data_ptr()
                            q.dx, q.lddx = dx.data_ptr(), dx.stride(0)
                            q.dgamma, q.dbeta = gmap[id(bn.weight)].data_ptr(), gmap[id(bn.bias)].data_ptr()
                        else:
                            q.dbn, q.lddbn = dx.data_ptr(), dx.stride(0)
                P.big_lin[train].append(q)

    def _prolog(self, L, idx, train):
        p = float(L.pro_drop.p) if (L.pro_drop is not None) else 0.0
        mask = self.dropout_masks.get(idx)
        return ops.inprolog(L.pro_bn, train=train, drop_p=p, drop_mask=mask, rng=self.rng, stream_id=idx + 1)

    def _opts_arg(self, P):
        o = ops.persistent_opts(self.dn_opts, self.device, 1, P.B, P.dims)
        self._opts_live = o
        return ctypes.byref(o)

    def _forward(self, P, train, enc_opts=None):
        self.sync_packs()
        P.fwd_serial += 1
        st = ops.stream()
        lib, prog = self.lib, self.prog
        B, (D, H, W) = P.B, (P.dims if P.has_enc else (1, 1, 1))
        if P.has_enc:
            feats = P.buf["feats"]
            out = feats[:, prog["ct_cols"]:]
            if P.fallback:
                self._check_scalar_path(P)
                _lib.check(lib.mms_fb3_forward(P.ws.data_ptr(), P.ws_bytes, P.widths, B, D, H, W, P.ct.data_ptr(), P.ptab, P.btab, out.data_ptr(),
                                               feats.stride(0), 1 if train else 0, st), "mms_fb3_forward")
            else:
                _lib.check(lib.mms_dn121_forward(P.ws.data_ptr(), B, D, H, W, P.ct.data_ptr(), P.ptab, P.btab, out.data_ptr(),
                                                 feats.stride(0), 1 if train else 0, enc_opts if enc_opts is not None else self._opts_arg(P), st),
                           "mms_dn121_forward")
        if P.big:
            if train:
                P.big_stats.zero_()
            bl, n_pre = P.big_lin[train], prog["n_pre"]
            for q in bl[:n_pre]:
                _lib.check(lib.mms_linear_big_fwd(ctypes.byref(q), st), "mms_linear_big_fwd")
            if P.gate is not None:
                self.entropy.zero_()
                _lib.check(lib.mms_gate_fwd(ctypes.byref(P.gate), st), "mms_gate_fwd")
            if P.mix is not None:
                _lib.check(lib.mms_missing_mix_fwd(ctypes.byref(P.mix), st), "mms_missing_mix_fwd")
            for q in bl[n_pre:]:
                _lib.check(lib.mms_linear_big_fwd(ctypes.byref(q), st), "mms_linear_big_fwd")
            return
        lf = P.lin_fwd[train]
        n_pre = prog["n_pre"]
        for i in range(n_pre):
            _lib.check(lib.mms_linear_fwd(ctypes.byref(lf[i]), st), "mms_linear_fwd")
        if P.moe is not None:
            _lib.check(lib.mms_moe_fwd(ctypes.byref(P.moe[0]), st), "mms_moe_fwd")
        if P.gate is not None:
            self.entropy.zero_()
            _lib.check(lib.mms_gate_fwd(ctypes.byref(P.gate), st), "mms_gate_fwd")
        if P.mix is not None:
            _lib.check(lib.mms_missing_mix_fwd(ctypes.byref(P.mix), st), "mms_missing_mix_fwd")
        for i in range(n_pre, len(lf)):
            _lib.check(lib.mms_linear_fwd(ctypes.byref(lf[i]), st), "mms_linear_fwd")
        if P.moe is not None:
            _lib.check(lib.mms_moe_fwd(ctypes.byref(P.moe[1]), st), "mms_moe_fwd")

    def _check_scalar_path(self, P):
        if not scalar_widths_ok(P.widths):
            raise ValueError("3-conv CT encoder widths %s: one model at a time runs the scalar kernels, which take widths that divide 256 "
                             "(16, 32, 64, 128); train and evaluate this model as a FoldGroupEngine (a group of one is fine)" % (tuple(P.widths),))

    def _backward_from_dhz(self, P):
        self._backward_heads(P)
        self._backward_encoder(P)

    def _backward_heads(self, P):
        st = ops.stream()
        lib, prog = self.lib, self.prog
        B, (D, H, W) = P.B, (P.dims if P.has_enc else (1, 1, 1))
        n_pre = prog["n_pre"]
        if P.big:
            def big_bwd(i):
                L, q = prog["lins"][i], P.big_lin[True][i]
                _lib.check(lib.mms_linear_big_bwd_w(ctypes.byref(q), st), "mms_linear_big_bwd_w")
                if L.need_dx:
                    _lib.check(lib.mms_linear_big_bwd_x(ctypes.byref(q), st), "mms_linear_big_bwd_x")
                    if L.pro_bn is not None:
                        _lib.check(lib.mms_bn1d_bwd_apply(ctypes.byref(q), st), "mms_bn1d_bwd_apply")
            for i in range(len(prog["lins"]) - 1, n_pre - 1, -1):
                big_bwd(i)
            if P.gate is not None:
                _lib.check(lib.mms_gate_bwd(ctypes.byref(P.gate), st), "mms_gate_bwd")
            if P.mix is not None:
                _lib.check(lib.mms_missing_mix_bwd(ctypes.byref(P.mix), st), "mms_missing_mix_bwd")
            for i in range(n_pre - 1, -1, -1):
                big_bwd(i)
            return
        if P.moe is not None:
            _lib.check(lib.mms_moe_bwd(ctypes.byref(P.moe_bwd[1]), st), "mms_moe_bwd")
        for i in range(len(P.lin_bwd) - 1, n_pre - 1, -1):
            _lib.check(lib.mms_linear_bwd(ctypes.byref(P.lin_bwd[i]), st), "mms_linear_bwd")
        if P.gate is not None:
            _lib.check(lib.mms_gate_bwd(ctypes.byref(P.gate), st), "mms_gate_bwd")
        if P.mix is not None:
            _lib.check(lib.mms_missing_mix_bwd(ctypes.byref(P.mix), st), "mms_missing_mix_bwd")
        if P.moe is not None:
            _lib.check(lib.mms_moe_bwd(ctypes.byref(P.moe_bwd[0]), st), "mms_moe_bwd")
        for i in range(n_pre - 1, -1, -1):
            _lib.check(lib.mms_linear_bwd(ctypes.byref(P.lin_bwd[i]), st), "mms_linear_bwd")

    def _backward_encoder(self, P, stage=None, hook=None):
        if not P.has_enc:
            return
        st = ops.stream()
        lib, prog = self.lib, self.prog
        B, (D, H, W) = P.B, P.dims
        dfe = P.dbuf["feats"]
        dct = dfe[:, prog["ct_cols"]:]
        if stage is not None or hook is not None or P.bn_world > 1:
            hi, lo = stage if stage is not None else (3, 0)
            _lib.check(lib.mms_dn121_backward_stage(P.ws.data_ptr(), B, D, H, W, P.ct.data_ptr(), P.ptab, dct.data_ptr(), dfe.stride(0),
                                                    P.gtab, hi, lo, P.bn_world, hook, None, self._opts_arg(P), st), "mms_dn121_backward_stage")
            return
        if os.environ.get("MMS_SIDE_STREAM") != "1" and not P.fallback:
            _lib.check(lib.mms_dn121_backward(P.ws.data_ptr(), B, D, H, W, P.ct.data_ptr(), P.ptab, dct.data_ptr(),
                                              dfe.stride(0), P.gtab, self._opts_arg(P), st), "mms_dn121_backward")
            return
        if P.fallback:
            _lib.check(lib.mms_fb3_backward(P.ws.data_ptr(), P.ws_bytes, P.widths, B, D, H, W, P.ct.data_ptr(), P.ptab, dct.data_ptr(),
                                            dfe.stride(0), P.gtab, st), "mms_fb3_backward")
            return
        _lib.check(lib.mms_dn121_backward_mt(P.ws.data_ptr(), B, D, H, W, P.ct.data_ptr(), P.ptab, dct.data_ptr(),
                                             dfe.stride(0), P.gtab, self._opts_arg(P), st, ctypes.c_void_p(self.side_stream.cuda_stream),
                                             ctypes.c_void_p(self.ev_fork.cuda_event), ctypes.c_void_p(self.ev_join.cuda_event)),
                   "mms_dn121_backward_mt")

    def _global_cox_buffers(self, P, world):
        if getattr(P, "gcox", None) is None or P.gcox["world"] != world:
            n, dev = world * P.B, self.device
            G = dict(world=world, h=torch.zeros(n, device=dev), time=torch.zeros(n, device=dev), event=torch.zeros(n, device=dev),
                     valid=torch.ones(n, device=dev), lse=torch.zeros(n, device=dev), dh=torch.zeros(n, device=dev), rank=0,
                     frac=torch.zeros(n, device=dev))
            G["cox"] = _S()["CoxP"](G["h"].data_ptr(), 1, G["time"].data_ptr(), G["event"].data_ptr(), G["valid"].data_ptr(), n, 1.0,
                                    G["lse"].data_ptr(), G["dh"].data_ptr(), 1, P.cox_out.data_ptr(), self.tie_mode, G["frac"].data_ptr())
            P.gcox = G
        return P.gcox

    def _train_body(self, P, skip_if_unusable, part="all"):
        st = ops.stream()
        lib = self.lib
        if part == "fwd":
            self.gflat.zero_()
            self.sumsq.zero_()
            self._forward(P, True)
            return
        if part in ("coxbwd", "coxheads"):
            G = P.gcox
            _lib.check(lib.mms_cox_fwd_bwd(ctypes.byref(G["cox"]), st), "mms_cox_fwd_bwd")
            P.dbuf["hz"][:, 0].copy_(G["dh"][G["rank"] * P.B:(G["rank"] + 1) * P.B])
            if part == "coxheads":
                self._backward_heads(P)
            else:
                self._backward_from_dhz(P)
            return
        if part == "gradheads":
            self.gflat.zero_()
            self.sumsq.zero_()
            self._forward(P, True)
            _lib.check(lib.mms_cox_fwd_bwd(ctypes.byref(P.cox), st), "mms_cox_fwd_bwd")
            self._backward_heads(P)
            return
        if isinstance(part, tuple) and part[0] == "enc":
            self._backward_encoder(P, stage=None if part[1] is None else (part[1], part[1]))
            return
        if isinstance(part, tuple) and part[0] == "update":
            if part[1] != 1.0:
                self.gflat.mul_(part[1])
            part = "update"
        if part in ("all", "grad"):
            self.gflat.zero_()
            self.sumsq.zero_()
            self._forward(P, True)
            self._cox_step(P)
            self._backward_from_dhz(P)
            if part == "grad":
                return
        if part == "update":
            self.sumsq.zero_()
        ad = P.adam_skip if skip_if_unusable else P.adam
        _lib.check(lib.mms_grad_sumsq(ctypes.byref(ad), st), "mms_grad_sumsq")
        _lib.check(lib.mms_clip_adam(ctypes.byref(ad), st), "mms_clip_adam")

    def load_batch(self, P, ct=None, rna=None, clinical=None, mask=None, time=None, event=None, valid=None, shared_ct=False):
        if P.has_enc and not shared_ct:
            P.ct.copy_(ct.reshape(P.ct.shape), non_blocking=True)
        if "rna" in P.buf:
            P.buf["rna"].copy_(rna, non_blocking=True)
        if clinical is not None and "clin" in P.buf:
            P.buf["clin"].copy_(clinical.reshape(P.buf["clin"].shape), non_blocking=True)
        if mask is not None:
            (P.mask2 if P.mix is not None else P.mask).copy_(mask, non_blocking=True)
        if time is not None:
            P.time.copy_(time.reshape(-1), non_blocking=True)
            P.event.copy_(event.reshape(-1).to(torch.float32), non_blocking=True)
        if valid is None:
            P.valid.fill_(1.0)
        else:
            P.valid.copy_(valid.reshape(-1).to(torch.float32), non_blocking=True)

    def gather_block(self, P, cohort, idx_dev, fold=None):
        G, _ = self._gather_sources(P, cohort, idx_dev, fold)
        return G

    def gather_aug_blocks(self, P, cohort, idx_dev, rec_dev, aff_dev=None, fold=None):
        from . import augment
        G, roles = self._gather_sources(P, cohort, idx_dev, fold)
        dims = tuple(P.ct.shape[-3:]) if P.has_enc else None
        A = augment.aug_block(rec_dev, roles, dims, (0, 0, 0))
        return (G, A) if aff_dev is None else (G, A, augment.aff_block(aff_dev))

    def _gather_sources(self, P, cohort, idx_dev, fold=None):
        from .augment import ROLE_MASK, ROLE_PLAIN, ROLE_VOLUME
        G = _S()["GatherP"]()
        G.idx, G.B = idx_dev.data_ptr(), P.B
        flags = {}
        if "mask" in cohort:
            chk = cohort.setdefault("_absent_rows_zero", {})
            for j, key in enumerate(("image", "rnaseq")):
                if key not in chk:
                    gone = cohort["mask"][:, j] == 0
                    chk[key] = bool((cohort[key][gone] == 0).all()) if bool(gone.any()) else True
                if chk[key]:
                    flags[key] = cohort["mask"][:, j:]
        srcs = []
        if "rna" in P.buf:
            rna = cohort["rnaseq"]
            if "rnaseq_folds" in cohort:
                from .gene_select import fold_matrix
                rna = fold_matrix(cohort, fold)
            if rna.shape[1] != P.buf["rna"].shape[1]:
                raise ValueError("the model reads %d RNA-seq columns, the cohort's matrix has %d" % (P.buf["rna"].shape[1], rna.shape[1]))
            srcs.append((rna, P.buf["rna"], None, flags.get("rnaseq"), ROLE_PLAIN, 1))
        if P.has_enc:
            srcs.append((cohort["image"].view(cohort["image"].shape[0], -1), P.ct.view(P.B, -1), None, flags.get("image"), ROLE_VOLUME, 0))
        if "clin" in P.buf:
            srcs.append((cohort["clinical"], P.buf["clin"], None, None, ROLE_PLAIN, 2))
        if P.gate is not None or P.moe is not None:
            srcs.append((cohort["mask"], P.mask, None, None, ROLE_MASK, -1))
        if P.mix is not None:
            srcs.append((cohort["mask"], P.mask2, P.mask2.shape[1], None, ROLE_MASK, -1))
        lab = cohort["label"]
        srcs.append((lab, P.time.view(P.B, 1), 1, None, ROLE_PLAIN, -1))
        srcs.append((lab[:, 1:], P.event.view(P.B, 1), 1, None, ROLE_PLAIN, -1))
        if "valid" in cohort:
            srcs.append((cohort["valid"].view(-1, 1), P.valid.view(P.B, 1), 1, None, ROLE_PLAIN, -1))
        G.nsrc = len(srcs)
        for i, (a, b, w, flag, _, _) in enumerate(srcs):
            if a.dtype != torch.float32 or not (a.is_cuda or a.is_pinned()):
                raise TypeError("gather sources must be fp32 tensors in device or pinned host memory")
            G.src[i], G.dst[i] = a.data_ptr(), b.data_ptr()
            G.src_ld[i], G.dst_ld[i] = a.stride(0), b.stride(0)
            G.width[i] = w if w is not None else a.shape[1]
            if flag is not None:
                G.present[i], G.present_ld[i] = flag.data_ptr(), flag.stride(0)
        return G, [(role, bit) for *_, role, bit in srcs]

    def train_step(self, ct=None, rna=None, clinical=None, mask=None, time=None, event=None, valid=None, skip_if_unusable=True,
                   use_graph=True, ddp_world=1, global_cox=False, sync_bn=False):
        B = (rna if rna is not None else ct).shape[0]
        self.check_train_batch(B, tuple(ct.shape[-3:]) if ct is not None else None, ddp_world if sync_bn else 1)
        P = self.plan(B, tuple(ct.shape[-3:]) if ct is not None else None, bn_world=ddp_world if (sync_bn and ddp_world > 1) else 1)
        self.load_batch(P, ct, rna, clinical, mask, time, event, valid)
        self.sync_packs()
        P.fwd_serial += 1
        if ddp_world > 1 and P.big and self.prog["encoder"] is not None:
            raise RuntimeError("the data-parallel steps of the imaging models are limited to 32 rows per rank (their staged graphs are "
                               "built and tested on the small-batch head kernels); got %d -- lower the per-rank batch (the global batch is "
                               "ddp_world times it) or train large batches on one GPU" % B)
        if ddp_world > 1 and P.moe is not None:
            raise RuntimeError("SimMLM_SurvivalNet: the data-parallel step (ddp_world > 1) is not implemented for this model; "
                               "train its folds as a fold group or one per process instead")
        if ddp_world > 1 and sync_bn:
            self._ddp_step_syncbn(P, ddp_world)
            return
        if ddp_world > 1:
            self._ddp_step(P, ddp_world, global_cox, use_graph)
            return
        if not use_graph:
            self._train_body(P, skip_if_unusable)
            return
        key = ("train", skip_if_unusable)
        if key not in P.graphs:
            P.graphs[key] = capture([self], lambda: self._train_body(P, skip_if_unusable))
        P.graphs[key].replay()

    def _buckets(self, P):
        if getattr(self, "_bucket_cache", None) is None:
            from . import distributed as D
            enc = self.prog["encoder"]
            staged = enc is not None and not isinstance(enc, nn.Sequential)
            self._bucket_cache = (staged, D.gradient_buckets(self.params, list(enc.parameters()) if enc is not None else [], staged))
        return self._bucket_cache

    def _ddp_sequence(self, P, global_cox):
        staged, buckets = self._buckets(P)
        seq = [("part", "fwd"), ("gather",), ("part", "coxheads")] if global_cox else [("part", "gradheads")]
        if staged:
            seq.append(("bucket", 0))
            for k, b in enumerate((3, 2, 1, 0)):
                seq += [("part", ("enc", b)), ("bucket", k + 1)]
        else:
            seq += [("part", ("enc", None)), ("bucket", 0)]
        return seq + [("wait",)], buckets

    def _ddp_step(self, P, world, global_cox, use_graph):
        from . import distributed as D
        import torch.distributed as dist
        seq, buckets = self._ddp_sequence(P, global_cox)
        upd = ("update", 1.0 if global_cox else 1.0 / world)
        if global_cox:
            G = self._global_cox_buffers(P, world)
            G["rank"] = dist.get_rank() if dist.is_initialized() else 0

        def run(run_part):
            works = []
            for item in seq:
                if item[0] == "part":
                    run_part(item[1])
                elif item[0] == "gather":
                    D.all_gather_into(G["h"], P.buf["hz"][:, 0], world)
                    D.all_gather_into(G["time"], P.time, world); D.all_gather_into(G["event"], P.event, world)
                    D.all_gather_into(G["valid"], P.valid, world)
                elif item[0] == "bucket":
                    works.append(D.allreduce_ranges_async(self.gflat, buckets[item[1]], world))
                else:
# ... 222 lines not shown
```

multimodal_survival_prediction_amd/fold_group.py:

```python
import ctypes

import torch

from . import _lib, ops
from .engine import SurvivalEngine, capture, check_attribute, gate_out, group_widths_ok

_S = _lib.structs


def _arr(blocks):
    T = type(blocks[0])
    return (T * len(blocks))(*blocks)


def _ptrs(vals):
    return (ctypes.c_void_p * len(vals))(*vals)


class _GroupPlan:
    pass


class FoldGroupEngine:
    MAX = 10

    FUSED_IMG_TAIL = True

    def __init__(self, models, fused_tail=None, folds=None, **engine_kw):
        self.folds = list(range(len(models))) if folds is None else [int(f) for f in folds]
        if len(self.folds) != len(models):
            raise ValueError("folds must name one fold per model")
        self.fused_tail = self.FUSED_IMG_TAIL if fused_tail is None else bool(fused_tail)
        if not 1 <= len(models) <= self.MAX:
            raise ValueError("a fold group holds 1..%d models" % self.MAX)
        self.lib = _lib.load_library()
        dev = next(models[0].parameters()).device
        if dev.type != "cuda":
            raise RuntimeError("FoldGroupEngine: models must be on the GPU (no CPU fallback)")
        n = sum(p.numel() for p in models[0].parameters())
        n += (-n) % 4
        G = len(models)
        self.device = dev
        self.gflat_all = torch.zeros(G, n, device=dev)
        self.sumsq_all = torch.zeros(G, dtype=torch.float64, device=dev)
        self.entropy_all = torch.zeros(G, device=dev)
        self.engines = []
        for g, m in enumerate(models):
            if getattr(m, "_mms_engine", None) is not None:
                raise RuntimeError("model %d already has an engine; build the group from fresh models" % g)
            if sum(p.numel() for p in m.parameters()) + (-sum(p.numel() for p in m.parameters())) % 4 != n:
                raise ValueError("fold-group models must have identical shapes")
            slots = dict(gflat=self.gflat_all[g], sumsq=self.sumsq_all[g:g + 1], entropy=self.entropy_all[g:g + 1])
            self.engines.append(SurvivalEngine(m, _slots=slots, **engine_kw))
        kinds = {e.prog["kind"] for e in self.engines}
        if len(kinds) != 1:
            raise ValueError("fold-group models must be of one class, got %s" % sorted(kinds))
        if len({bytes(e.dn_opts) for e in self.engines}) != 1:
            raise ValueError("fold-group models must share one encoder shape (class_layers.out width) and launch options")
        self.plans = {}

    def __len__(self):
        return len(self.engines)

    def plan(self, B, dims, members=None):
        members = self._members(members)
        key = (B,) + (tuple(dims) if dims is not None else ()) + (members,)
        if key in self.plans:
            return self.plans[key]
        if B > 32:
            raise RuntimeError("fold groups batch the small-batch head kernels, limited to 32 rows per model; got %d -- train "
                               "larger batches with one engine per fold (SurvivalEngine.train_step, fold after fold)" % B)
        eng = [self.engines[i] for i in members]
        Ps = [e.plan(B, dims) for e in eng]
        GP = _GroupPlan()
        GP.fallback = bool(Ps[0].has_enc and Ps[0].fallback)
        GP.members, GP.eng, GP.Ps, GP.B, GP.dims = members, eng, Ps, B, (tuple(dims) if dims is not None else ())
        prog = eng[0].prog
        GP.ng = len(eng)
        GP.has_enc = Ps[0].has_enc
        if GP.has_enc:
            GP.ws = _ptrs([P.ws.data_ptr() for P in Ps])
            GP.x = _ptrs([P.ct.data_ptr() for P in Ps])
            GP.params = _ptrs([ctypes.addressof(P.ptab) for P in Ps])
            GP.buffers = _ptrs([ctypes.addressof(P.btab) for P in Ps])
            GP.grads = _ptrs([ctypes.addressof(P.gtab) for P in Ps])
            cc = prog["ct_cols"]
            GP.out = _ptrs([P.buf["feats"][:, cc:].data_ptr() for P in Ps])
            GP.dout = _ptrs([P.dbuf["feats"][:, cc:].data_ptr() for P in Ps])
            GP.ld = Ps[0].buf["feats"].stride(0)
            if GP.fallback:
                GP.widths, GP.ws_bytes = Ps[0].widths, Ps[0].ws_bytes
                if any(tuple(P.widths) != tuple(GP.widths) for P in Ps):
                    raise ValueError("fold-group models must share the CT encoder's channel widths")
                if not group_widths_ok(GP.widths):
                    raise ValueError("3-conv CT encoder widths %s: the fold-group kernels take multiples of 16 other than 48 and 112" % (tuple(GP.widths),))
        GP.img_tail = bool(self.fused_tail and GP.fallback and prog["kind"] == "ImageOnlyModel")
        GP.mix = _arr([P.mix for P in Ps]) if Ps[0].mix is not None else None
        nl = len(prog["lins"])
        GP.lin_fwd = {t: [_arr([P.lin_fwd[t][i] for P in Ps]) for i in range(nl)] for t in (True, False)}
        GP.lin_bwd = [_arr([P.lin_bwd[i] for P in Ps]) for i in range(nl)]
        GP.gate = _arr([P.gate for P in Ps]) if Ps[0].gate is not None else None
        GP.moe = GP.moe_bwd = GP.cox4 = None
        if Ps[0].moe is not None:
            GP.moe = [_arr([P.moe[s] for P in Ps]) for s in (0, 1)]
            GP.moe_bwd = [_arr([P.moe_bwd[s] for P in Ps]) for s in (0, 1)]
            terms = [P.cox4[c] for P in Ps for c in range(4)]
            GP.cox4 = [(_arr(terms[i:i + 8]), len(terms[i:i + 8])) for i in range(0, len(terms), 8)]
        GP.cox = _arr([P.cox for P in Ps])
        GP.cox_eval = _arr([P.cox_eval for P in Ps])
        GP.adam = {True: _arr([P.adam_skip for P in Ps]), False: _arr([P.adam for P in Ps])}
        GP.graphs = {}
        GP.full = members == tuple(range(len(self.engines)))
        self.plans[key] = GP
        return GP

    def _forward(self, GP, train, x=None, enc_opts=None, img_tail=None):
        st = ops.stream()
        lib, ng = self.lib, GP.ng
        prog = GP.eng[0].prog
        if GP.has_enc:
            x = GP.x if x is None else x
            B, (D, H, W) = GP.B, GP.dims
            if GP.img_tail and img_tail is not False:
                lf = GP.lin_fwd[train]
                _lib.check(lib.mms_img_forward_group(ng, GP.ws, GP.ws_bytes, GP.widths, B, D, H, W, x, GP.params, GP.buffers, GP.out, GP.ld,
                                                     1 if train else 0, lf[0], lf[1], st), "mms_img_forward_group")
                return
            if GP.fallback:
                _lib.check(lib.mms_fb3_forward_group(ng, GP.ws, GP.ws_bytes, GP.widths, B, D, H, W, x, GP.params, GP.buffers, GP.out, GP.ld,
                                                     1 if train else 0, st), "mms_fb3_forward_group")
            else:
                _lib.check(lib.mms_dn121_forward_group(ng, GP.ws, B, D, H, W, x, GP.params, GP.buffers, GP.out, GP.ld,
                                                       1 if train else 0, enc_opts if enc_opts is not None else self._opts_arg(GP), st),
                           "mms_dn121_forward_group")
        self._forward_heads(GP, train)

    def _forward_heads(self, GP, train):
        st = ops.stream()
        lib, ng = self.lib, GP.ng
        prog = GP.eng[0].prog
        lf = GP.lin_fwd[train]
        n_pre = prog["n_pre"]
        for i in range(n_pre):
            _lib.check(lib.mms_linear_fwd_group(lf[i], ng, st), "mms_linear_fwd_group")
        if GP.moe is not None:
            _lib.check(lib.mms_moe_fwd_group(GP.moe[0], ng, st), "mms_moe_fwd_group")
        if GP.gate is not None:
            _lib.check(lib.mms_gate_fwd_group(GP.gate, ng, st), "mms_gate_fwd_group")
        if GP.mix is not None:
            _lib.check(lib.mms_missing_mix_fwd_group(GP.mix, ng, st), "mms_missing_mix_fwd_group")
        for i in range(n_pre, len(lf)):
            _lib.check(lib.mms_linear_fwd_group(lf[i], ng, st), "mms_linear_fwd_group")
        if GP.moe is not None:
            _lib.check(lib.mms_moe_fwd_group(GP.moe[1], ng, st), "mms_moe_fwd_group")

    @staticmethod
    def _sync_packs(GP):
        if GP.fallback:
            return
        for e in GP.eng:
            e.sync_packs()

    def _zero(self, GP):
        if GP.full:
            self.gflat_all.zero_(); self.sumsq_all.zero_(); self.entropy_all.zero_()
        else:
            for e in GP.eng:
                e.gflat.zero_(); e.sumsq.zero_(); e.entropy.zero_()

    def _train_body(self, GP, skip_if_unusable):
        st = ops.stream()
        lib, ng = self.lib, GP.ng
        prog = GP.eng[0].prog
        self._zero(GP)
        self._forward(GP, True)
        if GP.cox4 is not None:
            for arr, n in GP.cox4:
                _lib.check(lib.mms_cox_fwd_bwd_group(arr, n, st), "mms_cox_fwd_bwd_group")
            _lib.check(lib.mms_moe_bwd_group(GP.moe_bwd[1], ng, st), "mms_moe_bwd_group")
        else:
            _lib.check(lib.mms_cox_fwd_bwd_group(GP.cox, ng, st), "mms_cox_fwd_bwd_group")
        self._backward_from_dhz(GP)
        ad = GP.adam[bool(skip_if_unusable)]
        _lib.check(lib.mms_grad_sumsq_group(ad, ng, st), "mms_grad_sumsq_group")
        _lib.check(lib.mms_clip_adam_group(ad, ng, st), "mms_clip_adam_group")

    def _backward_from_dhz(self, GP):
        st = ops.stream()
        lib, ng = self.lib, GP.ng
        prog = GP.eng[0].prog
        if GP.img_tail:
            B, (D, H, W) = GP.B, GP.dims
            _lib.check(lib.mms_img_backward_group(ng, GP.ws, GP.ws_bytes, GP.widths, B, D, H, W, GP.x, GP.params, GP.grads,
                                                  GP.lin_bwd[0], GP.lin_bwd[1], st), "mms_img_backward_group")
            return
        n_pre = prog["n_pre"]
        for i in range(len(GP.lin_bwd) - 1, n_pre - 1, -1):
            _lib.check(lib.mms_linear_bwd_group(GP.lin_bwd[i], ng, st), "mms_linear_bwd_group")
        if GP.gate is not None:
            _lib.check(lib.mms_gate_bwd_group(GP.gate, ng, st), "mms_gate_bwd_group")
        if GP.mix is not None:
            _lib.check(lib.mms_missing_mix_bwd_group(GP.mix, ng, st), "mms_missing_mix_bwd_group")
        if GP.moe is not None:
            _lib.check(lib.mms_moe_bwd_group(GP.moe_bwd[0], ng, st), "mms_moe_bwd_group")
        for i in range(n_pre - 1, -1, -1):
            _lib.check(lib.mms_linear_bwd_group(GP.lin_bwd[i], ng, st), "mms_linear_bwd_group")
        if GP.has_enc:
            B, (D, H, W) = GP.B, GP.dims
            if GP.fallback:
                _lib.check(lib.mms_fb3_backward_group(ng, GP.ws, GP.ws_bytes, GP.widths, B, D, H, W, GP.x, GP.params, GP.dout, GP.ld, GP.grads, st),
                           "mms_fb3_backward_group")
            else:
                _lib.check(lib.mms_dn121_backward_group(ng, GP.ws, B, D, H, W, GP.x, GP.params, GP.dout, GP.ld, GP.grads, self._opts_arg(GP), st),
                           "mms_dn121_backward_group")

    def _opts_arg(self, GP):
        o = ops.persistent_opts(GP.eng[0].dn_opts, self.device, GP.ng, GP.B, GP.dims)
        GP.opts_live = o
        return ctypes.byref(o)

    def _graph(self, GP, key, body):
        if key not in GP.graphs:
            GP.graphs[key] = capture(GP.eng, body)
        return GP.graphs[key]

    def _members(self, members):
        return tuple(range(len(self.engines))) if members is None else tuple(members)

    @staticmethod
    def _rows(batch):
        return (batch["rna"] if batch.get("rna") is not None else batch["ct"]).shape[0]

    def _step(self, GP, skip_if_unusable, use_graph):
        self._sync_packs(GP)
        if not use_graph:
            self._train_body(GP, skip_if_unusable)
            return
        self._graph(GP, ("train", bool(skip_if_unusable)), lambda: self._train_body(GP, skip_if_unusable)).replay()

    def train_step(self, batches, members=None, skip_if_unusable=True, use_graph=True):
        members = self._members(members)
        if len(batches) != len(members):
            raise ValueError("one batch per member")
        has_enc = self.engines[0].prog["encoder"] is not None
        B = self._rows(batches[0])
        dims = tuple(batches[0]["ct"].shape[-3:]) if has_enc else None
        self.engines[0].check_train_batch(B, dims)
        for b in batches:
            if self._rows(b) != B or (has_enc and tuple(b["ct"].shape[-3:]) != dims):
                raise ValueError("fold-group batches must share one shape; split ragged tails into their own step")
        GP = self.plan(B, dims, members)
        for e, P, b in zip(GP.eng, GP.Ps, batches):
            e.load_batch(P, **b)
        self._step(GP, skip_if_unusable, use_graph)

    def _gather_indexed(self, GP, cohort, idx, augment=None, affine=None):
        members, B = GP.members, GP.B
        key = id(cohort)
        cache = GP.__dict__.setdefault("gather", {})
        if key not in cache:
            dev_idx = torch.zeros(len(members), B, dtype=torch.int64, device=self.device)
            pin = dict(bufs=[torch.zeros(len(members), B, dtype=torch.int64).pin_memory() for _ in range(4)],
                       evs=[None] * 4, k=0)
            blocks = _arr([e.gather_block(P, cohort, dev_idx[g], fold=self.folds[GP.members[g]]) for g, (e, P) in enumerate(zip(GP.eng, GP.Ps))])
            for e, P in zip(GP.eng, GP.Ps):
                if "valid" not in cohort:
                    P.valid.fill_(1.0)
            cache[key] = (dev_idx, pin, blocks, cohort)
        dev_idx, pin, blocks, _ = cache[key]
        if affine is not None and augment is None:
            raise ValueError("affine records come with the 8-word records of the same rows (augment=)")
        if augment is not None:
            aug = self._aug_blocks(GP, cohort, dev_idx, pin, augment, affine)
        k = pin["k"]
        pin["k"] = (k + 1) % len(pin["bufs"])
        if pin["evs"][k] is not None:
            pin["evs"][k].synchronize()
        pin["bufs"][k].copy_(idx)
        dev_idx.copy_(pin["bufs"][k], non_blocking=True)
        if augment is not None:
            aug["pin"][k].copy_(augment)
            aug["dev"].copy_(aug["pin"][k], non_blocking=True)
        if affine is not None:
            aug["aff_pin"][k].copy_(affine)
            aug["aff_dev"].copy_(aug["aff_pin"][k], non_blocking=True)
        ev = torch.cuda.Event()
        ev.record()
        pin["evs"][k] = ev
        if affine is not None:
            _lib.check(self.lib.mms_gather_affine_group(aug["gather"], aug["aug"], aug["aff"], GP.ng, ops.stream()), "mms_gather_affine_group")
            return
        if augment is not None:
            _lib.check(self.lib.mms_gather_aug_group(aug["gather"], aug["aug"], GP.ng, ops.stream()), "mms_gather_aug_group")
            return
        _lib.check(self.lib.mms_gather_rows_group(blocks, GP.ng, ops.stream()), "mms_gather_rows_group")

    def _aug_blocks(self, GP, cohort, dev_idx, pin, augment, affine=None):
        from . import augment as A
        has_mask = all(P.gate is not None or P.moe is not None or P.mix is not None for P in GP.Ps)
        if tuple(augment.shape) != (len(GP.members), GP.B, A.REC_WORDS):
            raise ValueError("augment must be [len(members)][B] records of %d words, got %r for %d members of %d rows"
                             % (A.REC_WORDS, tuple(augment.shape), len(GP.members), GP.B))
        mx = A.check_records(augment, GP.dims if GP.has_enc else None, has_mask)
        if affine is not None:
            if tuple(affine.shape) != (len(GP.members), GP.B, A.AFF_WORDS):
                raise ValueError("augment_affine must be [len(members)][B] records of %d words, got %r for %d members of %d rows"
                                 % (A.AFF_WORDS, tuple(affine.shape), len(GP.members), GP.B))
            A.check_affine_records(affine)
            mx = [0, 0, 0]
        cache = GP.__dict__.setdefault("gather_aug", {})
        key = id(cohort)
        if key not in cache:
            dev = torch.zeros(len(GP.members), GP.B, A.REC_WORDS, dtype=torch.int32, device=self.device)
            pairs = [e.gather_aug_blocks(P, cohort, dev_idx[g], dev[g], fold=self.folds[GP.members[g]]) for g, (e, P) in enumerate(zip(GP.eng, GP.Ps))]
            cache[key] = dict(dev=dev, pin=[torch.zeros(dev.shape, dtype=torch.int32).pin_memory() for _ in pin["bufs"]],
                              gather=_arr([g for g, _ in pairs]), aug=_arr([a for _, a in pairs]))
        aug = cache[key]
        if affine is not None and "aff" not in aug:
            aug["aff_dev"] = torch.zeros(len(GP.members), GP.B, A.AFF_WORDS, dtype=torch.int32, device=self.device)
            aug["aff_pin"] = [torch.zeros(aug["aff_dev"].shape, dtype=torch.int32).pin_memory() for _ in pin["bufs"]]
            aug["aff"] = _arr([A.aff_block(aug["aff_dev"][g]) for g in range(GP.ng)])
# ... 151 lines not shown
```

multimodal_survival_prediction_amd/ops.py:

```python
import ctypes

import torch

from . import _lib


def _S():
    return _lib.structs()


def stream():
    return ctypes.c_void_p(torch.cuda.current_stream().cuda_stream)


def ptr(t):
    return None if t is None else t.data_ptr()


def dims3(d):
    return _S()["Dims3"](int(d[0]), int(d[1]), int(d[2]))


def bnsrc(gamma, beta, count, train, sum=None, sumsq=None, rmean=None, rvar=None, eps=1e-5):
    return _S()["BnSrc"](ptr(sum), ptr(sumsq), ptr(rmean), ptr(rvar), ptr(gamma), ptr(beta),
# ... 41 lines not shown
    call("mms_conv1_fwd", p, opts)


def conv3_fwd(y1, coords, dims, wp, out, bn, osum=None, osumsq=None, partial=None, nsplit=27, wfrag=False, opts=None):
    M = y1.shape[0]
    p = _S()["Conv3FwdP"](ptr(y1), ptr(coords), dims3(dims), M, ptr(wp), ptr(out), out.stride(0), bn,
                          ptr(osum), ptr(osumsq), ptr(partial), nsplit)
    p.wfrag = 1 if wfrag else 0
    call("mms_conv3_fwd", p, opts)


def conv0_fwd(x, in_dims, out_dims, coords, w, y, osum=None, osumsq=None):
    p = _S()["Conv0FwdP"](ptr(x), dims3(in_dims), dims3(out_dims), ptr(coords), y.shape[0], ptr(w), ptr(y),
                          ptr(osum), ptr(osumsq))
    call("mms_conv0_fwd", p)


def pool_fwd(y0, in_dims, out_dims, B, slab, argmax, bn, osum=None, osumsq=None):
    p = _S()["PoolFwdP"](ptr(y0), dims3(in_dims), dims3(out_dims), B, ptr(slab), slab.stride(0), ptr(argmax), bn,
                         ptr(osum), ptr(osumsq))
    call("mms_pool_fwd", p)


def head_fwd(slab, C, B, V, bn, w, bias, pooled, out):
    p = _S()["HeadFwdP"](ptr(slab), slab.stride(0), C, B, V, bn, ptr(w), ptr(bias), w.shape[0], ptr(pooled), ptr(out), out.stride(0))
    call("mms_head_fwd", p)


def pack_conv3(w):
    wpf = torch.empty(32 * 27 * 128, dtype=torch.float32, device=w.device)
    wpb = torch.empty(128 * 27 * 32, dtype=torch.float32, device=w.device)
    _lib.check(_lib.load_library().mms_pack_conv3(w.data_ptr(), wpf.data_ptr(), wpb.data_ptr(), stream()), "mms_pack_conv3")
    return wpf, wpb


def pack_conv3_frag(w):
    wff = torch.empty(32 * 27 * 128, dtype=torch.float32, device=w.device)
    wfb = torch.empty(128 * 27 * 32, dtype=torch.float32, device=w.device)
    _lib.check(_lib.load_library().mms_pack_conv3_frag(w.data_ptr(), wff.data_ptr(), wfb.data_ptr(), stream()), "mms_pack_conv3_frag")
    return wff, wfb


def bnbwd(s1, s2):
    return _S()["BnBwd"](ptr(s1), ptr(s2))


def conv3_bwd_data(dz, coords, dims, wpb, y1, bn, dbn, s1, s2, partial=None, nsplit=27, wfrag=False, opts=None):
    p = _S()["Conv3BwdDataP"](ptr(dz), dz.stride(0), ptr(coords), dims3(dims), y1.shape[0], ptr(wpb), ptr(y1), bn,
                              ptr(dbn), ptr(s1), ptr(s2), ptr(partial), nsplit)
    p.wfrag = 1 if wfrag else 0
    call("mms_conv3_bwd_data", p, opts)


def conv3_bwd_weight(y1, coords, dims, bn, dz, dw, msplit=1, tapmajor=False, opts=None, layout=None):
    p = _S()["Conv3BwdWP"](ptr(y1), ptr(coords), dims3(dims), y1.shape[0], bn, ptr(dz), dz.stride(0), ptr(dw), msplit,
                           layout if layout is not None else (1 if tapmajor else 0))
    call("mms_conv3_bwd_weight", p, opts)


def conv1_bwd(which, dyraw, M, N, x, K, bn_in, w, dw, dbn, s1, s2, y=None, bn_out=None, bb_out=None, pool=False,
              in_dims=(0, 0, 0), msplit=1, dgamma_out=None, dbeta_out=None, fuse_dx=None, fuse_accumulate=True, fuse_dgamma=None,
              fuse_dbeta=None, opts=None):
    S = _S()
    p = S["Conv1BwdP"]()
    p.dyraw, p.lddy = ptr(dyraw), dyraw.stride(0)
    p.y, p.ldy = (ptr(y), y.stride(0)) if y is not None else (None, 0)
    p.has_bn_out = 1 if bn_out is not None else 0
    p.bn_out = bn_out if bn_out is not None else bn_in
    p.bb_out = bb_out if bb_out is not None else S["BnBwd"](None, None)
    p.M, p.N = M, N
    p.x, p.ldx, p.K, p.bn_in = ptr(x), x.stride(0), K, bn_in
    setattr(p, "in", dims3(in_dims))
    p.w = ptr(w)
    p.pool = 1 if pool else 0
    p.dw = ptr(dw)
    p.dbn, p.lddbn = ptr(dbn), dbn.stride(0)
    p.s1, p.s2 = ptr(s1), ptr(s2)
    p.msplit = msplit
    p.dgamma_out, p.dbeta_out = ptr(dgamma_out), ptr(dbeta_out)
    if fuse_dx is not None:
        p.fuse_dx, p.fuse_lddx, p.fuse_accumulate = ptr(fuse_dx), fuse_dx.stride(0), 1 if fuse_accumulate else 0
        p.fuse_dgamma, p.fuse_dbeta = ptr(fuse_dgamma), ptr(fuse_dbeta)
    if which == "weight":
        call("mms_conv1_bwd_weight", p)
    else:
        call("mms_conv1_bwd_data", p, opts)


def bn_bwd_apply(dbn, x, dx, M, C, bn, bb, accumulate, dgamma, dbeta):
    p = _S()["BnBwdApplyP"](ptr(dbn), dbn.stride(0), ptr(x), x.stride(0), ptr(dx), dx.stride(0), M, C, bn, bb,
                            1 if accumulate else 0, ptr(dgamma), ptr(dbeta))
    call("mms_bn_bwd_apply", p)


def head_bwd(dout, pooled, slab, C, B, V, bn, w, dw, dbias, dgamma, dbeta, dslab):
    p = _S()["HeadBwdP"](ptr(dout), dout.stride(0), ptr(pooled), ptr(slab), slab.stride(0), C, B, V, bn, ptr(w), w.shape[0],
                         ptr(dw), ptr(dbias), ptr(dgamma), ptr(dbeta), ptr(dslab), dslab.stride(0))
    call("mms_head_bwd", p)


def pool_bwd(dslab, argmax, out_dims, in_dims, B, y0, bn, dbn, s1, s2, coords=None):
    p = _S()["PoolBwdP"](ptr(dslab), dslab.stride(0), ptr(argmax), dims3(out_dims), dims3(in_dims), B, ptr(y0), bn,
                         ptr(dbn), ptr(s1), ptr(s2), ptr(coords))
    call("mms_pool_bwd", p)


def pool_act(x, K, bn, in_dims, y):
    p = _S()["PoolActP"](ptr(x), x.stride(0), K, bn, dims3(in_dims), y.shape[0], ptr(y), y.stride(0))
    _lib.check(_lib.load_library().mms_pool_act_group(ctypes.byref(p), 1, stream()), "mms_pool_act_group")


def conv0_bwd_weight(dbn, y0, bn, bb, x, in_dims, out_dims, coords, dw, msplit, dgamma, dbeta, dw_rep=None):
    p = _S()["Conv0BwdWP"](ptr(dbn), ptr(y0), bn, bb, ptr(x), dims3(in_dims), dims3(out_dims), ptr(coords),
                           y0.shape[0], ptr(dw), msplit, ptr(dgamma), ptr(dbeta), ptr(dw_rep), 0 if dw_rep is None else dw_rep.shape[0])
    call("mms_conv0_bwd_weight", p)


def conv0_bwd_data(dbn, bn, w, in_dims, out_dims, dx, group=None):
    S = _S()["Conv0BwdDataP"]
    mk = lambda d, b, w_, x_: S(ptr(d), b, ptr(w_), dims3(in_dims), dims3(out_dims), d.shape[0], ptr(x_))
    if group is None:
        call("mms_conv0_bwd_data", mk(dbn, bn, w, dx))
        return
    arr = (S * len(group))(*[mk(*m) for m in group])
    _lib.check(_lib.load_library().mms_conv0_bwd_data_group(arr, len(group), stream()), "mms_conv0_bwd_data_group")


def inprolog(bn=None, train=False, drop_p=0.0, drop_mask=None, rng=None, stream_id=0):
    S = _S()["InProlog"]
    if bn is None:
        return S(0, None, None, None, None, None, 1e-5, 0.1, 1 if train else 0, float(drop_p), ptr(drop_mask), ptr(rng), stream_id)
    return S(1, ptr(bn.weight), ptr(bn.bias), ptr(bn.running_mean), ptr(bn.running_var), ptr(bn.num_batches_tracked),
             float(bn.eps), float(bn.momentum), 1 if train else 0, float(drop_p), ptr(drop_mask), ptr(rng), stream_id)


def linear_fwd(x, K, pro, w, bias, y, out_relu):
    p = _S()["LinearFwdP"](ptr(x), x.stride(0), x.shape[0], K, pro, ptr(w), ptr(bias), w.shape[0], ptr(y), y.stride(0),
                           1 if out_relu else 0)
    call("mms_linear_fwd", p)


def linear_bwd(dy, y, out_relu, x, K, pro, w, dw, dbias, dx=None, dgamma=None, dbeta=None):
    p = _S()["LinearBwdP"](ptr(dy), dy.stride(0), ptr(y), y.stride(0), 1 if out_relu else 0, ptr(x), x.stride(0),
                           x.shape[0], K, pro, ptr(w), w.shape[0], ptr(dw), ptr(dbias), ptr(dx),
                           dx.stride(0) if dx is not None else 0, ptr(dgamma), ptr(dbeta))
    call("mms_linear_bwd", p)


def gate_params(feats, mask, w1, b1, w2, b2, hidden, gate, fused, dfused=None, ent_weight=0.0, dfeats=None,
                dw1=None, db1=None, dw2=None, db2=None, entropy=None, dgate_ext=None):
    return _S()["GateP"](ptr(feats), ptr(mask), feats.shape[0], ptr(w1), ptr(b1), ptr(w2), ptr(b2), ptr(hidden), ptr(gate),
                         ptr(fused), ptr(dfused), float(ent_weight), ptr(dgate_ext), ptr(dfeats), ptr(dw1), ptr(db1),
                         ptr(dw2), ptr(db2), ptr(entropy))


TIE_MODES = {"breslow": 0, "efron": 1}


def _cox_p(h, time, event, valid, scale, want_grad, ties):
    n = h.shape[0]
    lse = torch.empty(n, device=h.device)
    out = torch.empty(2, device=h.device)
    dh = torch.empty(n, device=h.device) if want_grad else None
    frac = torch.empty(n, device=h.device) if TIE_MODES[ties] == 1 else None
    p = _S()["CoxP"](ptr(h), h.stride(0), ptr(time), ptr(event), ptr(valid), n, float(scale), ptr(lse), ptr(dh), 1, ptr(out),
                     TIE_MODES[ties], ptr(frac))
    return p, out, dh, (lse, frac)


def cox_fwd_bwd(h, time, event, valid=None, scale=1.0, want_grad=True, ties="breslow"):
    p, out, dh, _scratch = _cox_p(h, time, event, valid, scale, want_grad, ties)
    call("mms_cox_fwd_bwd", p)
    return out, dh


def cox_fwd_bwd_group(members):
    built = [_cox_p(m["h"], m["time"], m["event"], m.get("valid"), m.get("scale", 1.0), True, m.get("ties", "breslow")) for m in members]
    arr = (_S()["CoxP"] * len(built))(*[b[0] for b in built])
    _lib.check(_lib.load_library().mms_cox_fwd_bwd_group(arr, len(built), stream()), "mms_cox_fwd_bwd_group")
    return [(b[1], b[2]) for b in built]


def cindex_counts(h, time, event):
    counts = torch.zeros(3, dtype=torch.int64, device=h.device)
    p = _S()["CindexP"](ptr(h), ptr(time), ptr(event), h.shape[0], ptr(counts))
    call("mms_cindex_counts", p)
    return counts


def cindex_boot(hrank, trank, event, w, stratum=None, pair_rule=0):
    hrank = hrank.reshape(1, -1) if hrank.dim() == 1 else hrank
    M, n = hrank.shape
    if w.dim() != 2 or w.shape[1] != n or w.dtype != torch.int8:
        raise ValueError("w must be int8 [R, n]")
    if trank.numel() != n or event.numel() != n or (stratum is not None and stratum.numel() != n):
        raise ValueError("trank / event / stratum must have n = %d elements" % n)
    dev = hrank.device
    i32 = lambda t: None if t is None else t.to(device=dev, dtype=torch.int32).contiguous()
    hrank, trank, event, stratum = i32(hrank), i32(trank), i32(event), i32(stratum)
    R, ldw = w.shape[0], (n + 63) // 64 * 64
    if ldw == n and w.is_contiguous() and w.data_ptr() % 16 == 0:
        wp = w
    else:
        wp = torch.zeros(R, ldw, dtype=torch.int8, device=dev)
        wp[:, :n] = w
    out = torch.zeros(M + 1, R, dtype=torch.int64, device=dev)
    p = _S()["CbootP"](ptr(hrank), n, M, ptr(trank), ptr(event), ptr(stratum), n, ptr(wp), ldw, R, ptr(out), int(pair_rule))
    call("mms_cindex_boot", p)
    return out


def gene_screen(x, off, row, coef, G=None, plan_only=False):
    import numpy as np
    if not (torch.is_tensor(x) and x.is_cuda and x.dtype == torch.float32 and x.dim() == 2 and x.stride(1) == 1):
        raise TypeError("x must be a 2-D fp32 device tensor with unit column stride")
    N, G = x.shape[0], x.shape[1] if G is None else int(G)
    off, row = np.asarray(off, dtype=np.int64).reshape(-1), np.asarray(row, dtype=np.int64).reshape(-1)
    coef = np.ascontiguousarray(np.asarray(coef, dtype=np.float64)).reshape(-1, 3)
    P = len(off) - 1
    if N < 1 or not 1 <= G <= x.shape[1]:
        raise ValueError("x must have N >= 1 rows and 1 <= G <= %d columns" % x.shape[1])
    if P < 0 or off[0] != 0 or (np.diff(off) < 0).any() or off[-1] != len(row) or len(coef) != len(row):
        raise ValueError("off must be non-decreasing from 0 to len(row) = len(coef)")
    if len(row) >= 2 ** 31:
        raise ValueError("the problems' row lists together must stay below 2^31 entries")
    if len(row) and (row.min() < 0 or row.max() >= N):
        raise ValueError("rows must lie in [0, %d)" % N)
    dev = x.device
    up = lambda a, dt: torch.from_numpy(np.ascontiguousarray(a.astype(dt) if len(a) else np.zeros(1, dt))).to(dev)
    off_d, row_d = up(off, np.int32), up(row, np.int32)
    coef_d = up(coef.reshape(-1), np.float64)
    U, V = torch.empty(max(P, 1), G, dtype=torch.float64, device=dev), torch.empty(max(P, 1), G, dtype=torch.float64, device=dev)
    p = _S()["GeneScreenP"](ptr(x), N, x.stride(0), G, P, ptr(off_d), ptr(row_d), ptr(coef_d), ptr(U), ptr(V))
    if plan_only:
        return p, (x, off_d, row_d, coef_d), U[:P], V[:P]
    call("mms_gene_screen", p)
    return U[:P], V[:P]


def logrank_scan(rank, pflag, coef, coff, cut, cset=None, at=None, tables=False, plan_only=False):
    import numpy as np
    dev = rank.device if torch.is_tensor(rank) and rank.is_cuda else torch.device("cuda")
    if not torch.is_tensor(rank):
        rank = torch.from_numpy(np.ascontiguousarray(np.asarray(rank, dtype=np.int32)))
    if rank.dim() != 2 or rank.dtype != torch.int32 or (rank.shape[0] and rank.shape[1] and rank.stride(1) != 1):
        raise TypeError("rank must be int32 [Q, n] with unit column stride")
    rank = rank.to(dev)
    Q, n = rank.shape
    if Q > 1 and rank.stride(0) < n:
        rank = rank.contiguous()
    pflag = np.asarray(pflag, dtype=np.int64).reshape(-1)
    coef = np.ascontiguousarray(np.asarray(coef, dtype=np.float64)).reshape(-1, 2)
    coff, cut = np.asarray(coff, dtype=np.int64).reshape(-1), np.asarray(cut, dtype=np.int64).reshape(-1)
    S = len(coff) - 1
    if n < 1 or len(pflag) != n or len(coef) != n:
        raise ValueError("rank must have n >= 1 columns, pflag n entries and coef [n, 2]")
    if ((pflag & ~3) != 0).any() or not np.array_equal((pflag & 2) != 0, (coef != 0).any(1)) or not np.isfinite(coef).all():
        raise ValueError("pflag must be [event] | 2 [coef != 0] and coef finite")
    if S < 0 or coff[0] != 0 or (np.diff(coff) < 0).any() or coff[-1] != len(cut):
        raise ValueError("coff must be non-decreasing from 0 to len(cut)")
    if len(cut) >= 2 ** 31 or (len(cut) and (np.abs(cut) >= 2 ** 31).any()):
        raise ValueError("cuts must be int32 and fewer than 2^31")
    inner = np.ones(len(cut), bool)
    inner[coff[:-1][coff[:-1] < len(cut)]] = False
    if len(cut) > 1 and ((np.diff(cut) < 0) & inner[1:]).any():
        raise ValueError("every cut set must be ascending")
    if cset is None:
        if S != Q:
            raise ValueError("without cset there is one cut set per problem: %d sets, %d problems" % (S, Q))
    else:
        cset = np.asarray(cset, dtype=np.int64).reshape(-1)
        if len(cset) != Q or (Q and (cset.min() < 0 or cset.max() >= S)):
            raise ValueError("cset must name one of the %d cut sets for each of the %d problems" % (S, Q))
    sizes = np.diff(coff)
    if at is not None:
        at = np.asarray(at, dtype=np.int64).reshape(-1)
        if len(at) != S or (at < -1).any() or (at >= sizes).any():
            raise ValueError("at must hold one cut index per set (-1: none)")
    maxc = int(sizes.max()) if S else 0
    up = lambda a, dt: torch.from_numpy(np.ascontiguousarray(a.astype(dt)).reshape(-1) if a.size else np.zeros(1, dt)).to(dev)
    t = dict(rank=rank if rank.numel() else torch.zeros(1, dtype=torch.int32, device=dev), pflag=up(pflag, np.int32),
             coef=up(coef, np.float64), coff=up(coff, np.int32), cut=up(cut, np.int32),
             cset=None if cset is None else up(cset, np.int32), at=None if at is None else up(at, np.int32))
    ldo = max(maxc, 1)
    out = dict(chi2_max=torch.zeros(max(Q, 1), dtype=torch.float64, device=dev), arg_max=torch.zeros(max(Q, 1), dtype=torch.int32, device=dev),
               chi2_at=torch.zeros(max(Q, 1), dtype=torch.float64, device=dev))
    if tables:
        out.update(U=torch.zeros(max(Q, 1), ldo, dtype=torch.float64, device=dev), V=torch.zeros(max(Q, 1), ldo, dtype=torch.float64, device=dev),
                   n_high=torch.zeros(max(Q, 1), ldo, dtype=torch.int32, device=dev), d_high=torch.zeros(max(Q, 1), ldo, dtype=torch.int32, device=dev))
    p = _S()["LogrankScanP"](n, max(rank.stride(0), n) if Q else n, Q, maxc, ptr(t["rank"]), ptr(t["pflag"]), ptr(t["coef"]), ptr(t["coff"]),
                             ptr(t["cut"]), ptr(t["cset"]), ptr(t["at"]), ptr(out["chi2_max"]), ptr(out["arg_max"]), ptr(out["chi2_at"]),
                             ptr(out.get("U")), ptr(out.get("V")), ptr(out.get("n_high")), ptr(out.get("d_high")), ldo)
    res = {k: (v[:Q, :maxc] if v.dim() == 2 else v[:Q]) for k, v in out.items()}
    if plan_only:
        return p, (t, out), res
    call("mms_logrank_scan", p)
    return res


def td_metrics(trank, event, hcut, rord, surv, w, plan_only=False):
    import numpy as np
    dev = next((t.device for t in (surv, w) if torch.is_tensor(t) and t.is_cuda), torch.device("cuda"))
    trank, event = np.asarray(trank, dtype=np.int64).reshape(-1), np.asarray(event, dtype=np.int64).reshape(-1)
    hcut, rord = np.asarray(hcut, dtype=np.int64).reshape(-1), np.asarray(rord, dtype=np.int64)
    n, H = len(trank), len(hcut)
    if n < 1 or H < 1 or len(event) != n or rord.ndim != 2 or rord.shape[0] < 1 or rord.shape[1] != n:
# ... 277 lines not shown
```

Baseline: 3782.

## Fuse linear backward kernels, batch zeroing, cache Cox in LDS, register-tile gate

Linear backward now launches the dW and dX bodies from one kernel with a partitioned grid instead of two launches. Per-step zeroing of the gradient, sumsq and entropy buffers goes through a single multi-span zero kernel, replacing several torch zero_ calls. The gate forward preloads its weights into registers, the Cox path gains an LDS-resident variant for small n, and grad sumsq uses 1024-thread blocks. The main target is launch overhead and redundant global reads in the small head kernels, at the cost of higher register pressure and more code paths.

```diff
diff --git a/include/mmsurv.h b/include/mmsurv.h
--- a/include/mmsurv.h
+++ b/include/mmsurv.h
@@ -328,6 +328,10 @@
     int tie_mode;
     float* tie_frac;
 } CoxP;
+
+typedef struct MmsZeroSpan {
+    void* p; size_t bytes;
+} MmsZeroSpan;
 
 typedef struct CindexP {
     const float* h; const float* time; const float* event; int n;
@@ -680,12 +684,16 @@
 int mms_zero_regions_group(void* const* regions_dev, int ng, size_t bytes, hipStream_t s);
 int mms_linear_fwd_group(const LinearFwdP* p, int ng, hipStream_t s);
 int mms_linear_bwd_group(const LinearBwdP* p, int ng, hipStream_t s);
+int mms_linear_bwd_group_form(const LinearBwdP* p, int ng, int form, hipStream_t s);
 int mms_gate_fwd_group(const GateP* p, int ng, hipStream_t s);
 int mms_gate_bwd_group(const GateP* p, int ng, hipStream_t s);
 int mms_cox_fwd_bwd_group(const CoxP* p, int ng, hipStream_t s);
+int mms_cox_fwd_bwd_group_form(const CoxP* p, int ng, int form, hipStream_t s);
+int mms_zero_spans_group(const MmsZeroSpan* spans, int n, hipStream_t s);
 int mms_moe_fwd_group(const MoeP* p, int ng, hipStream_t s);
 int mms_moe_bwd_group(const MoeP* p, int ng, hipStream_t s);
 int mms_grad_sumsq_group(const AdamP* p, int ng, hipStream_t s);
+int mms_grad_sumsq_group_form(const AdamP* p, int ng, int form, hipStream_t s);
 int mms_clip_adam_group(const AdamP* p, int ng, hipStream_t s);
 int mms_w2_pack_group(const AdamP* p, int ng, hipStream_t s);
 int mms_dn121_forward_group(int ng, void* const* ws, int B, int D, int H, int W, const float* const* x,
diff --git a/multimodal_survival_prediction_amd/csrc/abi.hip b/multimodal_survival_prediction_amd/csrc/abi.hip
--- a/multimodal_survival_prediction_amd/csrc/abi.hip
+++ b/multimodal_survival_prediction_amd/csrc/abi.hip
@@ -4,7 +4,7 @@
 #define SZ(T) if (strcmp(name, #T) == 0) return (int)sizeof(T);
 extern "C" int mms_abi_sizeof(const char* name) {
     SZ(Dims3) SZ(MmsDnOpts) SZ(BnSrc) SZ(BnBwd) SZ(Conv1FwdP) SZ(Conv3FwdP) SZ(Conv0FwdP) SZ(PoolFwdP) SZ(PoolActP) SZ(HeadFwdP)
-    SZ(Conv3BwdDataP) SZ(Conv3BwdWP) SZ(Conv1BwdP) SZ(BnBwdApplyP) SZ(HeadBwdP) SZ(PoolBwdP) SZ(Conv0BwdWP) SZ(Conv0BwdDataP) SZ(InProlog) SZ(LinearFwdP) SZ(LinearBwdP) SZ(GateP) SZ(CoxP) SZ(CindexP) SZ(AdamP) SZ(FbConvP) SZ(FbPoolP) SZ(GatherP) SZ(AugRec) SZ(AugP) SZ(AffRec) SZ(AffP) SZ(MixP) SZ(LinBigP) SZ(MoeP) SZ(MmsWgradModel) SZ(MmsWgradMember) SZ(MmsWgradShape) SZ(EnsP) SZ(CbootP) SZ(GeneScreenP) SZ(CoxnetP) SZ(LogrankScanP) SZ(TdMetricsP) SZ(CoxNewtonP)
+    SZ(Conv3BwdDataP) SZ(Conv3BwdWP) SZ(Conv1BwdP) SZ(BnBwdApplyP) SZ(HeadBwdP) SZ(PoolBwdP) SZ(Conv0BwdWP) SZ(Conv0BwdDataP) SZ(InProlog) SZ(LinearFwdP) SZ(LinearBwdP) SZ(GateP) SZ(CoxP) SZ(CindexP) SZ(AdamP) SZ(FbConvP) SZ(FbPoolP) SZ(GatherP) SZ(AugRec) SZ(AugP) SZ(AffRec) SZ(AffP) SZ(MixP) SZ(LinBigP) SZ(MoeP) SZ(MmsWgradModel) SZ(MmsWgradMember) SZ(MmsWgradShape) SZ(EnsP) SZ(CbootP) SZ(GeneScreenP) SZ(CoxnetP) SZ(LogrankScanP) SZ(TdMetricsP) SZ(CoxNewtonP) SZ(MmsZeroSpan)
     return -1;
 }
 extern "C" int mms_abi_version(void) { return 3; }
diff --git a/multimodal_survival_prediction_amd/csrc/heads.hip b/multimodal_survival_prediction_amd/csrc/heads.hip
--- a/multimodal_survival_prediction_amd/csrc/heads.hip
+++ b/multimodal_survival_prediction_amd/csrc/heads.hip
@@ -142,9 +142,8 @@
 MMS_SINGLE(mms_linear_fwd, LinearFwdP)
 
 template <int MM, bool KS4>
-__global__ __launch_bounds__(256) void linear_bwd_w_kernel(const Grp<LinearBwdP> grp) {
-    const LinearBwdP& p = grp.p[blockIdx.z];
-    const int lane = threadIdx.x & 63, wave = threadIdx.x >> 6, n = KS4 ? (int)blockIdx.x : (int)blockIdx.x * 4 + wave;
+__device__ __forceinline__ void linear_bwd_w_body(const LinearBwdP& p, const int bx) {
+    const int lane = threadIdx.x & 63, wave = threadIdx.x >> 6, n = KS4 ? bx : bx * 4 + wave;
     if (n >= p.N) return;
     constexpr int KSTEP = KS4 ? 256 : 64;
     float dz[MM], db = 0.f;
@@ -194,12 +193,9 @@
 }
 
 template <int MM>
-__global__ __launch_bounds__(256) void linear_bwd_x_kernel(const Grp<LinearBwdP> grp) {
-    const LinearBwdP& p = grp.p[blockIdx.z];
-    __shared__ float dzs[MM][128];
-    __shared__ float red[3][MM][64];
+__device__ __forceinline__ void linear_bwd_x_body(const LinearBwdP& p, const int bx, float (&dzs)[MM][128], float (&red)[3][MM][64]) {
     const int lane = threadIdx.x & 63, wave = threadIdx.x >> 6;
-    const int k = blockIdx.x * 64 + lane;
+    const int k = bx * 64 + lane;
     const int N = p.N, K = p.K;
     const float* __restrict__ wk = p.w + (k < K ? k : K - 1);
     float acc[MM];
@@ -267,30 +263,57 @@
     for (int m = 0; m < MM; ++m) if (m < p.M) p.dx[(size_t)m * p.lddx + k] = dxv[m];
 }
 
+template <int MM, bool KS4>
+__global__ __launch_bounds__(256) void linear_bwd_w_kernel(const Grp<LinearBwdP> grp) {
+    linear_bwd_w_body<MM, KS4>(grp.p[blockIdx.z], (int)blockIdx.x);
+}
 template <int MM>
-static int launch_linear_bwd(const Grp<LinearBwdP>& a, int ng, hipStream_t s) {
+__global__ __launch_bounds__(256) void linear_bwd_x_kernel(const Grp<LinearBwdP> grp) {
+    __shared__ float dzs[MM][128];
+    __shared__ float red[3][MM][64];
+    linear_bwd_x_body<MM>(grp.p[blockIdx.z], (int)blockIdx.x, dzs, red);
+}
+template <int MM, bool KS4>
+__global__ __launch_bounds__(256) void linear_bwd_kernel(const Grp<LinearBwdP> grp, const int wgrid) {
+    const LinearBwdP& p = grp.p[blockIdx.z];
+    __shared__ float dzs[MM][128];
+    __shared__ float red[3][MM][64];
+    if ((int)blockIdx.x < wgrid) linear_bwd_w_body<MM, KS4>(p, (int)blockIdx.x);
+    else linear_bwd_x_body<MM>(p, (int)blockIdx.x - wgrid, dzs, red);
+}
+
+template <int MM>
+static int launch_linear_bwd(const Grp<LinearBwdP>& a, int ng, int form, hipStream_t s) {
     const LinearBwdP& p = a.p[0];
+    const bool ks4 = p.K >= 2048;
+    const int wgrid = ks4 ? p.N : (p.N + 3) / 4, xgrid = (p.K + 63) / 64;
+    if (p.dw && p.dx && form == 0) {
+        if (ks4) MMS_LAUNCH((linear_bwd_kernel<MM, true>), dim3(wgrid + xgrid, 1, ng), dim3(256), 0, s, a, wgrid);
+        else MMS_LAUNCH((linear_bwd_kernel<MM, false>), dim3(wgrid + xgrid, 1, ng), dim3(256), 0, s, a, wgrid);
+        return mms_check_launch();
+    }
     if (p.dw) {
-        if (p.K >= 2048) MMS_LAUNCH((linear_bwd_w_kernel<MM, true>), dim3(p.N, 1, ng), dim3(256), 0, s, a);
-        else MMS_LAUNCH((linear_bwd_w_kernel<MM, false>), dim3((p.N + 3) / 4, 1, ng), dim3(256), 0, s, a);
-    }
-    if (p.dx) MMS_LAUNCH(linear_bwd_x_kernel<MM>, dim3((p.K + 63) / 64, 1, ng), dim3(256), 0, s, a);
-    return mms_check_launch();
-}
-extern "C" int mms_linear_bwd_group(const LinearBwdP* pp, int ng, hipStream_t s) {
+        if (ks4) MMS_LAUNCH((linear_bwd_w_kernel<MM, true>), dim3(wgrid, 1, ng), dim3(256), 0, s, a);
+        else MMS_LAUNCH((linear_bwd_w_kernel<MM, false>), dim3(wgrid, 1, ng), dim3(256), 0, s, a);
+    }
+    if (p.dx) MMS_LAUNCH(linear_bwd_x_kernel<MM>, dim3(xgrid, 1, ng), dim3(256), 0, s, a);
+    return mms_check_launch();
+}
+extern "C" int mms_linear_bwd_group_form(const LinearBwdP* pp, int ng, int form, hipStream_t s) {
     Grp<LinearBwdP> a;
-    if (!grp_fill(a, pp, ng, 1)) return MMS_ERR_ARG;
+    if (!grp_fill(a, pp, ng, 1) || form < 0 || form > 1) return MMS_ERR_ARG;
     const LinearBwdP& p = *pp;
     if (p.M <= 0 || p.M > 32 || p.N <= 0 || p.K <= 0) return MMS_ERR_ARG;
     for (int g = 1; g < ng; ++g) {
         const LinearBwdP& q = pp[g];
         if (q.M != p.M || q.N != p.N || q.K != p.K || (q.dw == nullptr) != (p.dw == nullptr) || (q.dx == nullptr) != (p.dx == nullptr)) return MMS_ERR_ARG;
     }
-    if (p.M <= 4) return launch_linear_bwd<4>(a, ng, s);
-    if (p.M <= 8) return launch_linear_bwd<8>(a, ng, s);
-    if (p.M <= 16) return launch_linear_bwd<16>(a, ng, s);
-    return launch_linear_bwd<32>(a, ng, s);
-}
+    if (p.M <= 4) return launch_linear_bwd<4>(a, ng, form, s);
+    if (p.M <= 8) return launch_linear_bwd<8>(a, ng, form, s);
+    if (p.M <= 16) return launch_linear_bwd<16>(a, ng, form, s);
+    return launch_linear_bwd<32>(a, ng, form, s);
+}
+extern "C" int mms_linear_bwd_group(const LinearBwdP* pp, int ng, hipStream_t s) { return mms_linear_bwd_group_form(pp, ng, 0, s); }
 MMS_SINGLE(mms_linear_bwd, LinearBwdP)
 
 #define GATE_F 288
@@ -301,20 +324,47 @@
     const GateP& p = grp.p[blockIdx.z];
     __shared__ float G[GATE_IN + 1], h[64], g[3];
     const int m = blockIdx.x, t = threadIdx.x, lane = t & 63, wave = t >> 6;
-    for (int i = t; i < GATE_IN; i += 256)
-        G[i] = i < GATE_F ? p.feats[(size_t)m * GATE_F + i] * p.mask[m * 3 + gate_seg(i)] : p.mask[m * 3 + (i - GATE_F)];
-    __syncthreads();
-    for (int j = wave * 16; j < wave * 16 + 16; ++j) {
+    constexpr int NK = (GATE_IN + 63) / 64;
+    float wv[16][NK];
+#pragma unroll
+    for (int u = 0; u < 16; ++u)
+#pragma unroll
+        for (int i = 0; i < NK; ++i) {
+            const int k = lane + 64 * i;
+            wv[u][i] = p.w1[(wave * 16 + u) * GATE_IN + (k < GATE_IN ? k : GATE_IN - 1)];
+        }
+    const float b1v = p.b1[wave * 16 + (lane & 15)];
+    float w2v[3], b2v[3];
+#pragma unroll
+    for (int c = 0; c < 3; ++c) { w2v[c] = p.w2[c * 64 + lane]; b2v[c] = p.b2[c]; }
+    {
+        const int i1 = t + 256;
+        const float f0 = p.feats[(size_t)m * GATE_F + t], m0 = p.mask[m * 3 + gate_seg(t)];
+        const float f1 = p.feats[(size_t)m * GATE_F + (i1 < GATE_F ? i1 : 0)];
+        const float m1 = p.mask[m * 3 + (i1 < GATE_F ? gate_seg(i1) : (i1 < GATE_IN ? i1 - GATE_F : 0))];
+        G[t] = f0 * m0;
+        if (i1 < GATE_IN) G[i1] = i1 < GATE_F ? f1 * m1 : m1;
+        else if (i1 == GATE_IN) G[i1] = 0.f;
+    }
+    __syncthreads();
+    float gk[NK];
+#pragma unroll
+    for (int i = 0; i < NK; ++i) gk[i] = G[lane + 64 * i < GATE_IN ? lane + 64 * i : GATE_IN];
+    float mine = 0.f;
+#pragma unroll
+    for (int u = 0; u < 16; ++u) {
         float a = 0.f;
-        for (int k = lane; k < GATE_IN; k += 64) a = fmaf(p.w1[j * GATE_IN + k], G[k], a);
+#pragma unroll
+        for (int i = 0; i < NK; ++i) if (lane + 64 * i < GATE_IN) a = fmaf(wv[u][i], gk[i], a);
         a = wave_sum(a);
-        if (lane == 0) { h[j] = fmaxf(a + p.b1[j], 0.f); p.hidden[m * 64 + j] = h[j]; }
-    }
+        if (lane == u) mine = a;
+    }
+    if (lane < 16) { const float hv = fmaxf(mine + b1v, 0.f); h[wave * 16 + lane] = hv; p.hidden[m * 64 + wave * 16 + lane] = hv; }
     __syncthreads();
     if (wave == 0) {
         float l[3];
 #pragma unroll
-        for (int c = 0; c < 3; ++c) l[c] = wave_sum(p.w2[c * 64 + lane] * h[lane]) + p.b2[c];
+        for (int c = 0; c < 3; ++c) l[c] = wave_sum(w2v[c] * h[lane]) + b2v[c];
         if (lane == 0) {
             const float mx = fmaxf(l[0], fmaxf(l[1], l[2]));
             const float e0 = expf(l[0] - mx), e1 = expf(l[1] - mx), e2 = expf(l[2] - mx), inv = 1.f / (e0 + e1 + e2);
@@ -496,99 +546,208 @@
 
 __device__ __forceinline__ bool cox_valid(const CoxP& p, int i) { return p.valid == nullptr || p.valid[i] != 0.f; }
 
+struct CoxMem {
+    const CoxP& p;
+    __device__ __forceinline__ bool valid(int i) const { return cox_valid(p, i); }
+    __device__ __forceinline__ float time(int i) const { return p.time[i]; }
+    __device__ __forceinline__ float event(int i) const { return p.event[i]; }
+    __device__ __forceinline__ float h(int i) const { return p.h[(size_t)i * p.ldh]; }
+    __device__ __forceinline__ float lse(int i) const { return p.lse[i]; }
+    __device__ __forceinline__ float frac(int i) const { return p.tie_frac[i]; }
+    __device__ __forceinline__ void put_lse(int i, float v) const { p.lse[i] = v; }
+    __device__ __forceinline__ void put_frac(int i, float v) const { p.tie_frac[i] = v; }
+};
+#define COX_ONE_N 256
+struct CoxLds {
+    const CoxP& p;
+    float (&t)[COX_ONE_N]; float (&e)[COX_ONE_N]; float (&hh)[COX_ONE_N]; float (&v)[COX_ONE_N]; float (&l)[COX_ONE_N]; float (&f)[COX_ONE_N];
+    __device__ __forceinline__ bool valid(int i) const { return v[i] != 0.f; }
+    __device__ __forceinline__ float time(int i) const { return t[i]; }
+    __device__ __forceinline__ float event(int i) const { return e[i]; }
+    __device__ __forceinline__ float h(int i) const { return hh[i]; }
+    __device__ __forceinline__ float lse(int i) const { return l[i]; }
+    __device__ __forceinline__ float frac(int i) const { return f[i]; }
+    __device__ __forceinline__ void put_lse(int i, float x) const { l[i] = x; p.lse[i] = x; }
+    __device__ __forceinline__ void put_frac(int i, float x) const { f[i] = x; p.tie_frac[i] = x; }
+};
+
+template <class S>
+__device__ __forceinline__ void cox_lse_row(const CoxP& p, const S& src, const int i, const int lane) {
+    if (!src.valid(i)) { if (lane == 0) { src.put_lse(i, 0.f); if (p.tie_mode == 1) src.put_frac(i, -1.f); } return; }
+    const float ti = src.time(i);
+    float mx = -INFINITY;
+    for (int j = lane; j < p.n; j += 64)
+        if (src.valid(j) && src.time(j) >= ti) mx = fmaxf(mx, src.h(j));
+    mx = wave_max(mx);
+    float s = 0.f;
+    if (p.tie_mode != 1) {
+        for (int j = lane; j < p.n; j += 64)
+            if (src.valid(j) && src.time(j) >= ti) s += expf(src.h(j) - mx);
+        s = wave_sum(s);
+        if (lane == 0) src.put_lse(i, mx + logf(s));
+        return;
+    }
+    float st = 0.f, m = 0.f, l = 0.f;
+    for (int j = lane; j < p.n; j += 64)
+        if (src.valid(j)) {
+            const float tj = src.time(j);
+            if (tj >= ti) {
+                const float e = expf(src.h(j) - mx);
+                s += e;
+                if (tj == ti && src.event(j) != 0.f) { st += e; m += 1.f; l += j < i ? 1.f : 0.f; }
+            }
+        }
+    s = wave_sum(s); st = wave_sum(st); m = wave_sum(m); l = wave_sum(l);
+    if (lane == 0) {
+        const bool ev = src.event(i) != 0.f;
+        const float f = ev ? l / m : 0.f;
+        src.put_lse(i, mx + logf(s - f * st));
+        src.put_frac(i, ev ? f : -1.f);
+    }
+}
+
+template <class S>
+__device__ __forceinline__ void cox_counts(const CoxP& p, const S& src, float* red, const bool first, bool& usable, float& denom) {
+    const int lane = threadIdx.x & 63, wave = threadIdx.x >> 6;
+    const bool efron = p.tie_mode == 1;
+    float nv = 0.f, ne = 0.f, ls = 0.f, nd = 0.f;
+    for (int j = threadIdx.x; j < p.n; j += 256)
+        if (src.valid(j)) {
+            nv += 1.f;
+            if (src.event(j) != 0.f) {
+                ne += 1.f; ls += src.h(j) - src.lse(j);
+                if (efron && src.frac(j) == 0.f) nd += 1.f;
+            }
+        }
+    nv = wave_sum(nv); ne = wave_sum(ne); ls = wave_sum(ls); nd = wave_sum(nd);
+    if (lane == 0) { red[wave] = nv; red[4 + wave] = ne; }
+    __syncthreads();
+    nv = red[0] + red[1] + red[2] + red[3]; ne = red[4] + red[5] + red[6] + red[7];
+    __syncthreads();
+    if (lane == 0) { red[wave] = ls; red[4 + wave] = nd; }
+    __syncthreads();
+    ls = red[0] + red[1] + red[2] + red[3]; nd = red[4] + red[5] + red[6] + red[7];
+    usable = nv >= 2.f && ne > 0.f;
+    denom = efron ? nd : ne + 1e-8f;
+    if (first && threadIdx.x == 0) {
+        p.out[0] = usable ? -ls / denom : 0.f;
+        p.out[1] = usable ? 1.f : 0.f;
+    }
+}
+template <class S>
+__device__ __forceinline__ void cox_grad_row(const CoxP& p, const S& src, const int k, const int lane, const bool usable, const float denom) {
+    const bool efron = p.tie_mode == 1;
+    float gsum = 0.f;
+    if (usable && src.valid(k)) {
+        const float tk = src.time(k), hk = src.h(k);
+        const bool ek = src.event(k) != 0.f;
+        for (int i = lane; i < p.n; i += 64)
+            if (src.valid(i) && src.event(i) != 0.f && src.time(i) <= tk) {
+                float w = 1.f;
+                if (efron && ek && src.time(i) == tk) w -= src.frac(i);
+                gsum += w * expf(hk - src.lse(i));
+            }
+        gsum = wave_sum(gsum);
+        if (lane == 0) p.dh[(size_t)k * p.lddh] = -p.scale * ((ek ? 1.f : 0.f) - gsum) / denom;
+    } else if (lane == 0) {
+        p.dh[(size_t)k * p.lddh] = 0.f;
+    }
+}
+
 __global__ __launch_bounds__(256) void cox_lse_kernel(const Grp<CoxP> grp) {
     const CoxP& p = grp.p[blockIdx.z];
     const int lane = threadIdx.x & 63, i = blockIdx.x * 4 + (threadIdx.x >> 6);
     if (i >= p.n) return;
-    if (!cox_valid(p, i)) { if (lane == 0) { p.lse[i] = 0.f; if (p.tie_mode == 1) p.tie_frac[i] = -1.f; } return; }
-    const float ti = p.time[i];
-    float mx = -INFINITY;
-    for (int j = lane; j < p.n; j += 64)
-        if (cox_valid(p, j) && p.time[j] >= ti) mx = fmaxf(mx, p.h[(size_t)j * p.ldh]);
-    mx = wave_max(mx);
-    float s = 0.f;
-    if (p.tie_mode != 1) {
-        for (int j = lane; j < p.n; j += 64)
-            if (cox_valid(p, j) && p.time[j] >= ti) s += expf(p.h[(size_t)j * p.ldh] - mx);
-        s = wave_sum(s);
-        if (lane == 0) p.lse[i] = mx + logf(s);
-        return;
-    }
-    float st = 0.f, m = 0.f, l = 0.f;
-    for (int j = lane; j < p.n; j += 64)
-        if (cox_valid(p, j)) {
-            const float tj = p.time[j];
-            if (tj >= ti) {
-                const float e = expf(p.h[(size_t)j * p.ldh] - mx);
-                s += e;
-                if (tj == ti && p.event[j] != 0.f) { st += e; m += 1.f; l += j < i ? 1.f : 0.f; }
-            }
-        }
-    s = wave_sum(s); st = wave_sum(st); m = wave_sum(m); l = wave_sum(l);
-    if (lane == 0) {
-        const bool ev = p.event[i] != 0.f;
-        const float f = ev ? l / m : 0.f;
-        p.lse[i] = mx + logf(s - f * st);
-        p.tie_frac[i] = ev ? f : -1.f;
-    }
-}
-
+    cox_lse_row(p, CoxMem{p}, i, lane);
+}
 __global__ __launch_bounds__(256) void cox_grad_kernel(const Grp<CoxP> grp) {
     const CoxP& p = grp.p[blockIdx.z];
     __shared__ float red[8];
-    const int lane = threadIdx.x & 63, wave = threadIdx.x >> 6, k = blockIdx.x * 4 + wave;
-    const bool efron = p.tie_mode == 1;
-    float nv = 0.f, ne = 0.f, ls = 0.f, nd = 0.f;
-    for (int j = threadIdx.x; j < p.n; j += 256)
-        if (cox_valid(p, j)) {
-            nv += 1.f;
-            if (p.event[j] != 0.f) {
-                ne += 1.f; ls += p.h[(size_t)j * p.ldh] - p.lse[j];
-                if (efron && p.tie_frac[j] == 0.f) nd += 1.f;
-            }
-        }
-    nv = wave_sum(nv); ne = wave_sum(ne); ls = wave_sum(ls); nd = wave_sum(nd);
-    if (lane == 0) { red[wave] = nv; red[4 + wave] = ne; }
-    __syncthreads();
-    nv = red[0] + red[1] + red[2] + red[3]; ne = red[4] + red[5] + red[6] + red[7];
-    __syncthreads();
-    if (lane == 0) { red[wave] = ls; red[4 + wave] = nd; }
-    __syncthreads();
-    ls = red[0] + red[1] + red[2] + red[3]; nd = red[4] + red[5] + red[6] + red[7];
-    const bool usable = nv >= 2.f && ne > 0.f;
-    const float denom = efron ? nd : ne + 1e-8f;
-    if (blockIdx.x == 0 && threadIdx.x == 0) {
-        p.out[0] = usable ? -ls / denom : 0.f;
-        p.out[1] = usable ? 1.f : 0.f;
-    }
+    const int lane = threadIdx.x & 63, k = blockIdx.x * 4 + (threadIdx.x >> 6);
+    bool usable; float denom;
+    cox_counts(p, CoxMem{p}, red, blockIdx.x == 0, usable, denom);
     if (k >= p.n || p.dh == nullptr) return;
-    float gsum = 0.f;
-    if (usable && cox_valid(p, k)) {
-        const float tk = p.time[k], hk = p.h[(size_t)k * p.ldh];
-        const bool ek = p.event[k] != 0.f;
-        for (int i = lane; i < p.n; i += 64)
-            if (cox_valid(p, i) && p.event[i] != 0.f && p.time[i] <= tk) {
-                float w = 1.f;
-                if (efron && ek && p.time[i] == tk) w -= p.tie_frac[i];
-                gsum += w * expf(hk - p.lse[i]);
-            }
-        gsum = wave_sum(gsum);
-        if (lane == 0) p.dh[(size_t)k * p.lddh] = -p.scale * ((ek ? 1.f : 0.f) - gsum) / denom;
-    } else if (lane == 0) {
-        p.dh[(size_t)k * p.lddh] = 0.f;
-    }
-}
-extern "C" int mms_cox_fwd_bwd_group(const CoxP* pp, int ng, hipStream_t s) {
+    cox_grad_row(p, CoxMem{p}, k, lane, usable, denom);
+}
+__global__ __launch_bounds__(256) void cox_one_kernel(const Grp<CoxP> grp) {
+    const CoxP& p = grp.p[blockIdx.z];
+    __shared__ float st[COX_ONE_N], se[COX_ONE_N], sh[COX_ONE_N], sv[COX_ONE_N], sl[COX_ONE_N], sf[COX_ONE_N], red[8];
+    const int t = threadIdx.x, lane = t & 63, wave = t >> 6;
+    if (t < p.n) {
+        st[t] = p.time[t]; se[t] = p.event[t]; sh[t] = p.h[(size_t)t * p.ldh];
+        sv[t] = p.valid ? p.valid[t] : 1.f;
+    }
+    __syncthreads();
+    const CoxLds src{p, st, se, sh, sv, sl, sf};
+    for (int i = wave; i < p.n; i += 4) cox_lse_row(p, src, i, lane);
+    __syncthreads();
+    bool usable; float denom;
+    cox_counts(p, src, red, true, usable, denom);
+    if (p.dh == nullptr) return;
+    for (int k = wave; k < p.n; k += 4) cox_grad_row(p, src, k, lane, usable, denom);
+}
+extern "C" int mms_cox_fwd_bwd_group_form(const CoxP* pp, int ng, int form, hipStream_t s) {
     Grp<CoxP> a;
-    if (!grp_fill(a, pp, ng, 1)) return MMS_ERR_ARG;
+    if (!grp_fill(a, pp, ng, 1) || form < 0 || form > 1) return MMS_ERR_ARG;
     const CoxP& p = *pp;
     for (int g = 0; g < ng; ++g)
         if (pp[g].n != p.n || pp[g].n <= 0 || !pp[g].lse || !pp[g].out || pp[g].tie_mode < 0 || pp[g].tie_mode > 1 || (pp[g].tie_mode == 1 && !pp[g].tie_frac)) return MMS_ERR_ARG;
+    if (form == 0 && p.n <= COX_ONE_N) {
+        MMS_LAUNCH(cox_one_kernel, dim3(1, 1, ng), dim3(256), 0, s, a);
+        return mms_check_launch();
+    }
     MMS_LAUNCH(cox_lse_kernel, dim3((p.n + 3) / 4, 1, ng), dim3(256), 0, s, a);
     MMS_LAUNCH(cox_grad_kernel, dim3((p.n + 3) / 4, 1, ng), dim3(256), 0, s, a);
     return mms_check_launch();
 }
+extern "C" int mms_cox_fwd_bwd_group(const CoxP* pp, int ng, hipStream_t s) { return mms_cox_fwd_bwd_group_form(pp, ng, 0, s); }
 MMS_SINGLE(mms_cox_fwd_bwd, CoxP)
+
+#define ZS_MAX (3 * MMS_MAX_GROUP)
+#define ZS_U 4
+#define ZS_WORDS (256 * ZS_U)
+struct ZeroSpans { MmsZeroSpan s[ZS_MAX]; unsigned first[ZS_MAX + 1]; int n; };
+__global__ __launch_bounds__(256) void zero_spans_kernel(const ZeroSpans a) {
+    int i = 0;
+    while (i + 1 < a.n && blockIdx.x >= a.first[i + 1]) ++i;
+    const unsigned lb = blockIdx.x - a.first[i];
+    unsigned char* const p = (unsigned char*)a.s[i].p;
+    const size_t bytes = a.s[i].bytes;
+    size_t head = (size_t)((16 - ((uintptr_t)p & 15)) & 15);
+    if (head > bytes) head = bytes;
+    const size_t words = (bytes - head) >> 4, tail = (bytes - head) & 15;
+    float4* const body = (float4*)(p + head);
+    const size_t w0 = (size_t)lb * ZS_WORDS + threadIdx.x;
+#pragma unroll
+    for (int u = 0; u < ZS_U; ++u) {
+        const size_t w = w0 + (size_t)u * 256;
+        if (w < words) body[w] = make_float4(0.f, 0.f, 0.f, 0.f);
+    }
+    if (lb == 0) {
+        if (threadIdx.x < head) p[threadIdx.x] = 0;
+        else if (threadIdx.x >= 16 && threadIdx.x - 16 < tail) p[head + (words << 4) + (threadIdx.x - 16)] = 0;
+    }
+}
+extern "C" int mms_zero_spans_group(const MmsZeroSpan* spans, int n, hipStream_t s) {
+    if (!spans || n < 1 || n > ZS_MAX) return MMS_ERR_ARG;
+    ZeroSpans a{};
+    unsigned long long blocks = 0;
+    for (int i = 0; i < n; ++i) {
+        if (!spans[i].p || spans[i].bytes == 0) return MMS_ERR_ARG;
+        a.s[i] = spans[i];
+        a.first[i] = (unsigned)blocks;
+        size_t head = (size_t)((16 - ((uintptr_t)spans[i].p & 15)) & 15);
+        if (head > spans[i].bytes) head = spans[i].bytes;
+        const size_t words = (spans[i].bytes - head) >> 4;
+        const size_t nb = (words + ZS_WORDS - 1) / ZS_WORDS;
+        blocks += nb ? nb : 1;
+        if (blocks > 0x7fffffffull) return MMS_ERR_ARG;
+    }
+    for (int i = n; i <= ZS_MAX; ++i) a.first[i] = (unsigned)blocks;
+    a.n = n;
+    MMS_LAUNCH(zero_spans_kernel, dim3((unsigned)blocks), dim3(256), 0, s, a);
+    return mms_check_launch();
+}
 
 __global__ __launch_bounds__(256) void cindex_kernel(const CindexP p) {
     const int lane = threadIdx.x & 63, i = blockIdx.x * 4 + (threadIdx.x >> 6);
@@ -615,12 +774,13 @@
     return mms_check_launch();
 }
 
-__global__ __launch_bounds__(256) void grad_sumsq_kernel(const Grp<AdamP> grp) {
+template <int T>
+__global__ __launch_bounds__(T) void grad_sumsq_kernel(const Grp<AdamP> grp) {
     const AdamP& p = grp.p[blockIdx.z];
-    __shared__ double red[4];
-    const long long n4 = p.n >> 2, stride = (long long)gridDim.x * 256;
+    __shared__ double red[T / 64];
+    const long long n4 = p.n >> 2, stride = (long long)gridDim.x * T;
     float a = 0.f, a1 = 0.f, a2 = 0.f, a3 = 0.f;
-    long long i = (long long)blockIdx.x * 256 + threadIdx.x;
+    long long i = (long long)blockIdx.x * T + threadIdx.x;
     for (; i + 3 * stride < n4; i += 4 * stride) {
         const float4 g0 = ((const float4*)p.g)[i], g1 = ((const float4*)p.g)[i + stride], g2 = ((const float4*)p.g)[i + 2 * stride],
                      g3 = ((const float4*)p.g)[i + 3 * stride];
@@ -783,15 +943,17 @@
     }
     return true;
 }
-extern "C" int mms_grad_sumsq_group(const AdamP* pp, int ng, hipStream_t s) {
+extern "C" int mms_grad_sumsq_group_form(const AdamP* pp, int ng, int form, hipStream_t s) {
     Grp<AdamP> a;
-    if (!adam_group(a, pp, ng)) return MMS_ERR_ARG;
+    if (!adam_group(a, pp, ng) || form < 0 || form > 1) return MMS_ERR_ARG;
     long long blocks = (pp->n / 16 + 255) / 256;
     if (blocks > 1024) blocks = 1024;
     if (blocks < 1) blocks = 1;
-    MMS_LAUNCH(grad_sumsq_kernel, dim3((unsigned)blocks, 1, ng), dim3(256), 0, s, a);
-    return mms_check_launch();
-}
+    if (form == 0 && (blocks & 3) == 0) MMS_LAUNCH(grad_sumsq_kernel<1024>, dim3((unsigned)(blocks >> 2), 1, ng), dim3(1024), 0, s, a);
+    else MMS_LAUNCH(grad_sumsq_kernel<256>, dim3((unsigned)blocks, 1, ng), dim3(256), 0, s, a);
+    return mms_check_launch();
+}
+extern "C" int mms_grad_sumsq_group(const AdamP* pp, int ng, hipStream_t s) { return mms_grad_sumsq_group_form(pp, ng, 0, s); }
 extern "C" int mms_clip_adam_group(const AdamP* pp, int ng, hipStream_t s) {
     Grp<AdamP> a;
     if (!adam_group(a, pp, ng)) return MMS_ERR_ARG;
diff --git a/multimodal_survival_prediction_amd/engine.py b/multimodal_survival_prediction_amd/engine.py
--- a/multimodal_survival_prediction_amd/engine.py
+++ b/multimodal_survival_prediction_amd/engine.py
@@ -563,7 +563,12 @@
         self._opts_live = o
         return ctypes.byref(o)
 
-    def _forward(self, P, train, enc_opts=None):
+    def _zero_step(self):
+        if getattr(self, "_zspans", None) is None:
+            self._zspans = ops.zero_spans([self.gflat, self.sumsq, self.entropy])
+        _lib.check(self.lib.mms_zero_spans_group(self._zspans, len(self._zspans), ops.stream()), "mms_zero_spans_group")
+
+    def _forward(self, P, train, enc_opts=None, entropy_zeroed=False):
         self.sync_packs()
         P.fwd_serial += 1
         st = ops.stream()
@@ -587,7 +592,8 @@
             for q in bl[:n_pre]:
                 _lib.check(lib.mms_linear_big_fwd(ctypes.byref(q), st), "mms_linear_big_fwd")
             if P.gate is not None:
-                self.entropy.zero_()
+                if not entropy_zeroed:
+                    self.entropy.zero_()
                 _lib.check(lib.mms_gate_fwd(ctypes.byref(P.gate), st), "mms_gate_fwd")
             if P.mix is not None:
                 _lib.check(lib.mms_missing_mix_fwd(ctypes.byref(P.mix), st), "mms_missing_mix_fwd")
@@ -601,7 +607,8 @@
         if P.moe is not None:
             _lib.check(lib.mms_moe_fwd(ctypes.byref(P.moe[0]), st), "mms_moe_fwd")
         if P.gate is not None:
-            self.entropy.zero_()
+            if not entropy_zeroed:
+                self.entropy.zero_()
             _lib.check(lib.mms_gate_fwd(ctypes.byref(P.gate), st), "mms_gate_fwd")
         if P.mix is not None:
             _lib.check(lib.mms_missing_mix_fwd(ctypes.byref(P.mix), st), "mms_missing_mix_fwd")
@@ -695,9 +702,8 @@
         st = ops.stream()
         lib = self.lib
         if part == "fwd":
-            self.gflat.zero_()
-            self.sumsq.zero_()
-            self._forward(P, True)
+            self._zero_step()
+            self._forward(P, True, entropy_zeroed=True)
             return
         if part in ("coxbwd", "coxheads"):
             G = P.gcox
@@ -709,9 +715,8 @@
                 self._backward_from_dhz(P)
             return
         if part == "gradheads":
-            self.gflat.zero_()
-            self.sumsq.zero_()
-            self._forward(P, True)
+            self._zero_step()
+            self._forward(P, True, entropy_zeroed=True)
             _lib.check(lib.mms_cox_fwd_bwd(ctypes.byref(P.cox), st), "mms_cox_fwd_bwd")
             self._backward_heads(P)
             return
@@ -723,9 +728,8 @@
                 self.gflat.mul_(part[1])
             part = "update"
         if part in ("all", "grad"):
-            self.gflat.zero_()
-            self.sumsq.zero_()
-            self._forward(P, True)
+            self._zero_step()
+            self._forward(P, True, entropy_zeroed=True)
             self._cox_step(P)
             self._backward_from_dhz(P)
             if part == "grad":
diff --git a/multimodal_survival_prediction_amd/fold_group.py b/multimodal_survival_prediction_amd/fold_group.py
--- a/multimodal_survival_prediction_amd/fold_group.py
+++ b/multimodal_survival_prediction_amd/fold_group.py
@@ -162,11 +162,13 @@
             e.sync_packs()
 
     def _zero(self, GP):
-        if GP.full:
-            self.gflat_all.zero_(); self.sumsq_all.zero_(); self.entropy_all.zero_()
-        else:
-            for e in GP.eng:
-                e.gflat.zero_(); e.sumsq.zero_(); e.entropy.zero_()
+        if getattr(GP, "zero_spans", None) is None:
+            if GP.full:
+                ts = [self.gflat_all, self.sumsq_all, self.entropy_all]
+            else:
+                ts = [t for e in GP.eng for t in (e.gflat, e.sumsq, e.entropy)]
+            GP.zero_spans = ops.zero_spans(ts)
+        _lib.check(self.lib.mms_zero_spans_group(GP.zero_spans, len(GP.zero_spans), ops.stream()), "mms_zero_spans_group")
 
     def _train_body(self, GP, skip_if_unusable):
         st = ops.stream()
diff --git a/multimodal_survival_prediction_amd/ops.py b/multimodal_survival_prediction_amd/ops.py
--- a/multimodal_survival_prediction_amd/ops.py
+++ b/multimodal_survival_prediction_amd/ops.py
@@ -217,6 +217,14 @@
     return _S()["GateP"](ptr(feats), ptr(mask), feats.shape[0], ptr(w1), ptr(b1), ptr(w2), ptr(b2), ptr(hidden), ptr(gate),
                          ptr(fused), ptr(dfused), float(ent_weight), ptr(dgate_ext), ptr(dfeats), ptr(dw1), ptr(db1),
                          ptr(dw2), ptr(db2), ptr(entropy))
+
+
+def zero_spans(tensors):
+    S = _S()["MmsZeroSpan"]
+    for t in tensors:
+        if not t.is_contiguous():
+            raise ValueError("zero_spans: contiguous tensors only")
+    return (S * len(tensors))(*[S(t.data_ptr(), t.numel() * t.element_size()) for t in tensors])
 
 
 TIE_MODES = {"breslow": 0, "efron": 1}
```

Result: faster. 3856 (median of 6 runs) (+2.0%).
